# Alpha-VLLM/Lumina-T2X

Measured on AMD Instinct MI355X. Metric: denoising-steps/s & latent-tokens/s, Next-DiT 2B 1024^2 CFG, higher is better.
Workload: dtype bf16

## Files before the change

### include/lumina_dit_debug.h

```cpp
#ifndef LUMINA_DIT_DEBUG_H
#define LUMINA_DIT_DEBUG_H

#include "lumina_dit.h"

#ifdef __cplusplus
extern "C" {
#endif


int lt_op_attention_trace(const void* q_dev, const void* k_dev, const void* vt_dev, void* out_dev, int32_t B,
                          int32_t H, int32_t Hkv, int32_t N, int32_t Nk, int32_t Nkpad, int32_t hd, float scale,
                          void* trace_dev, void* stream);

int lt_op_rmsnorm_mod_ex(const void* x, const void* w, const void* scale, const void* shift, int32_t ld_mod, void* out, int32_t B,
                         int32_t N, int32_t d, float eps, int32_t scale_pre, int32_t out_pair, void* stream);
int lt_op_gated_residual_norm_ex(void* x, const void* y, const void* post_w, const void* gate, int32_t post_mode, int32_t gate_mode,
                                 const void* next_w, const void* next_scale, const void* next_shift, int32_t next_mode, int32_t ld_mod,
                                 void* h, int32_t B, int32_t N, int32_t d, float eps, float eps_next, int32_t scale_pre, int32_t h_pair,
                                 const void* ystat, int32_t ystat_slots, const void* moe_ys, const void* moe_pos, const void* moe_wts,
                                 const void* route_w, int32_t route_E, void* route_sel, void* route_wts, const void* route_forced,
                                 void* stream);
int lt_op_gated_residual_norm_describe(int32_t post_mode, int32_t gate_mode, int32_t next_mode, int32_t d, int32_t has_next_w,
                                       int32_t has_next_scale, int32_t has_next_shift, int32_t scale_pre, int32_t has_ystat,
                                       int32_t ystat_slots, int32_t has_moe, char* out, int32_t cap);
// ... 9 lines not shown
int lt_op_qkv_post(const void* qkv, int32_t ld, int32_t q_col0, int32_t k_col0, int32_t v_col0, const void* q_ln_w, const void* q_ln_b,
                   const void* k_ln_w, const void* k_ln_b, float ln_eps, void* q_dst, void* k_dst, void* vt_dst, int32_t B, int32_t N,
                   int32_t Npad, int32_t heads, int32_t kv_heads, int32_t hd, int32_t rope_mode, const void* cs_table, int32_t cs_len,
                   const void* t, float watershed, int32_t grid_w, const void* n_tok_b, const void* grid_w_b, float q_out_scale,
                   float k_out_scale, void* stream);

int lt_op_rk_stage(const void* y_dev, const void* const* k_ptrs_host, const float* coef_host, int32_t nk, float dt, void* out_dev, int64_t n,
                   int32_t dtype, void* stream);
int lt_op_rk_error_norm(const void* y_dev, const void* y1_dev, const void* const* k_ptrs_host, const float* coef_host, int32_t nk, float dt,
                        float rtol, float atol, void* q_dev, void* ws_dev, float* norm_dev, int64_t n, int32_t dtype, void* stream);
int lt_op_rk_dense(const void* y_dev, const void* y1_dev, const void* ymid_dev, const void* fy_dev, const void* f1_dev, float dt, void* c1_dev,
                   void* c_dev, void* b_dev, void* a_dev, int64_t n, int32_t dtype, void* stream);
int lt_op_rk_interp(const void* const* coef_ptrs_host, float x, void* out_dev, int64_t n, int32_t dtype, void* stream);
int lt_op_rms_norm(const void* x_dev, const void* sub_dev, const void* y0_dev, float rtol, float atol, void* q_dev, void* ws_dev, float* norm_dev,
                   int64_t n, int32_t dtype, void* stream);

int lt_op_patchify(const void* x, int32_t x_dtype, void* out, int32_t B, int32_t C, int32_t H, int32_t W, int32_t patch, int32_t kpad,
                   int32_t dup_first_half, int32_t wp_stride, void* stream);
int lt_op_eol_fill(void* x, const void* eol, int32_t rows_total, int32_t Wp, int32_t d, void* stream);
int lt_op_fill_rows_bf16(void* dst, const void* row, int64_t rows, int32_t d, void* stream);
int lt_op_label_gather(const void* table, const void* labels, void* out, int32_t B, int32_t rows, int32_t d, void* stream);
int lt_op_cast_to_bf16(const void* src, int32_t dtype, void* dst, int64_t n, void* stream);
int lt_op_upload_rows(const void* src, int32_t dtype, void* dst, int32_t rows, int32_t cols, int32_t dst_ld, int32_t r0, int32_t row_map,
                      void* stream);
int lt_op_mask_to_bias(const void* mask, void* bias, int32_t B, int32_t T, int32_t Tpad, void* stream);
int lt_op_add_bf16(const void* a, const void* b, void* c, int64_t n, void* stream);
int lt_op_timestep_features(const void* t, int32_t t_index, void* out, int32_t B, int32_t dim, void* stream);
int lt_op_cap_pool_ln(const void* cap, int32_t cap_dtype, const void* mask, const void* ln_w, const void* ln_b, void* out, int32_t B, int32_t T,
                      int32_t C, void* stream);
int lt_op_unpatchify_cfg(const void* rows, int32_t ld, void* out, int32_t out_dtype, int32_t B, int32_t C, int32_t out_ch, int32_t H, int32_t W,
                         int32_t patch, int32_t use_cfg, float cfg_scale, int32_t cfg_channels, int32_t wp_stride, void* stream);
int lt_op_unpatchify_cfg_dev(const void* rows, int32_t ld, void* out, int32_t out_dtype, int32_t B, int32_t C, int32_t out_ch, int32_t H, int32_t W,
                             int32_t patch, int32_t use_cfg, const float* cfg_scale_dev, int32_t cfg_channels, int32_t wp_stride, int32_t dup,
                             void* stream);
int32_t lt_op_guidance_slices(void);
int lt_op_guidance_stats(const void* rows, int32_t ld, int32_t B, int32_t out_ch, int32_t H, int32_t W, int32_t patch, const float* cfg_scale_dev,
                         int32_t cfg_channels, int32_t wp_stride, double* partials_dev, void* stream);
int lt_op_unpatchify_cfg_rule(const void* rows, int32_t ld, void* out, int32_t out_dtype, int32_t B, int32_t C, int32_t out_ch, int32_t H, int32_t W,
                              int32_t patch, int32_t use_cfg, const float* cfg_scale_dev, int32_t cfg_channels, int32_t wp_stride, int32_t dup,
                              const double* partials_dev, const float* rescale_dev, const float* norm_limit_dev, float* factor_out_dev,
                              void* stream);
int lt_op_guidance_project_stats(const void* rows, int32_t ld, int32_t B, int32_t out_ch, int32_t H, int32_t W, int32_t patch, int32_t cfg_channels,
                                 int32_t wp_stride, int32_t form, const float* par_dev, float* mom_dev, double* partials_dev, void* stream);
int lt_op_unpatchify_cfg_project(const void* rows, int32_t ld, void* out, int32_t out_dtype, int32_t B, int32_t C, int32_t out_ch, int32_t H,
                                 int32_t W, int32_t patch, int32_t use_cfg, const float* cfg_scale_dev, int32_t cfg_channels, int32_t wp_stride,
                                 int32_t dup, int32_t form, const double* partials_dev, const float* par_dev, const float* mom_dev,
                                 float* coef_out_dev, void* stream);
int lt_op_unpatchify_cfg_reuse(const void* rows, int32_t ld, void* out, int32_t out_dtype, int32_t B, int32_t C, int32_t out_ch, int32_t H, int32_t W,
                               int32_t patch, const float* cfg_scale_dev, int32_t cfg_channels, int32_t wp_stride, void* delta_dev, int32_t mode,
                               void* stream);
int lt_op_unpatchify_cfg_slg(const void* rows, int32_t ld, void* out, int32_t out_dtype, int32_t B, int32_t C, int32_t out_ch, int32_t H, int32_t W,
                             int32_t patch, const float* cfg_scale_dev, const float* slg_scale_dev, int32_t cfg_channels, int32_t wp_stride,
                             void* skip_dev, int32_t mode, void* stream);
int lt_op_attention_identity(const void* src, int32_t ld_src, int32_t col0, void* out, int32_t B, int32_t N, int32_t H, int32_t Hkv, int32_t hd,
                             int32_t out_pair, void* stream);
int lt_debug_cache_read(lt_engine* e, int32_t which, void* dst_dev, int64_t n, void* stream);
int32_t lt_op_cache_ws_bytes(void);
int lt_op_cache_indicator(const void* h_dev, void* h_prev_dev, int64_t n, void* ws_dev, double* sums_dev, void* stream);
int lt_op_cache_residual_store(const void* xl_dev, const void* x0_dev, void* r_dev, int64_t n, void* stream);
int lt_op_cache_residual_apply(void* x_dev, const void* r_dev, const void* scale1p_dev, const void* shift_dev, int32_t ld_mod, void* h_dev, int32_t B,
                               int32_t N, int32_t d, void* stream);
int lt_op_packed_table(const int32_t* hw_host, int32_t B, int32_t C, int32_t patch, int32_t* table_host, int64_t* elems, int32_t* n_max);
int lt_op_patchify_packed(const void* x_flat, int32_t x_dtype, void* out, const int32_t* hw_host, void* tab_dev, int32_t B, int32_t C,
                          int32_t patch, int32_t kpad, int32_t N, int32_t dup_first_half, void* stream);
int lt_op_fill_pad_packed(void* x, const void* pad_token, const int32_t* hw_host, void* tab_dev, int32_t B, int32_t patch, int32_t N, int32_t d,
                          void* stream);
int lt_op_unpatchify_packed(const void* rows, int32_t ld, void* out_flat, int32_t out_dtype, const int32_t* hw_host, void* tab_dev, int32_t B,
                            int32_t C, int32_t out_ch, int32_t patch, int32_t N, int32_t use_cfg, float cfg_scale, int32_t cfg_channels,
                            void* stream);
int lt_op_region_text_combine(void* out, const void* txt, const void* gate, int32_t Y, int32_t N, int32_t H, int32_t hd, int32_t Hp, int32_t Wp,
                              int32_t h_split, int32_t w_split, void* stream);
int lt_op_ode_combine(int32_t mode, const void* y0, const void* k1, const void* k2, const void* k3, const void* k4, void* out, int32_t dtype,
                      float dt, int64_t n, void* stream);
int lt_op_ode_combine_masked(int32_t mode, const void* y0, const void* k1, const void* k2, const void* k3, const void* k4, const void* mask,
                             const void* x1, const void* noise, void* out, int32_t dtype, float dt, float t, float one_minus_t, int64_t n,
                             void* stream);
int lt_op_ode_multistep(const void* y_prev, const void* const* k, int32_t nslopes, const float* a, const float* b, int32_t has_corr, void* y_out,
                        void* p_out, int64_t n, int32_t dtype, void* stream);
int lt_op_rope_table(void* out, int32_t len, int32_t hd, int32_t step, float theta0, float lin0, float theta1, float lin1, int32_t lin_on_pos,
                     void* stream, void* out_t);
int lt_op_linear_small_m_ext(const void* a, const void* w, const void* b, void* y, int32_t M, int32_t N, int32_t K, int32_t act_in, const void* t,
                             const void* a2, int32_t pm_L, int32_t pm_chunks, int32_t pm_d, int32_t pm_final, uint32_t pm_tanh, uint32_t pm_scale,
                             void* stream);
int lt_op_moe_route(const void* x, const void* gate_w, const void* forced, int32_t rows, int32_t rows_per_sample, int32_t d, int32_t E, void* sel,
                    void* wts, int32_t max_tiles, void* stream);
int lt_op_moe_plan_ex(void* sel, const void* sample_logits, int32_t sample_ld, const void* forced, void* wts, int32_t rows,
                      int32_t rows_per_sample, int32_t E, void* pos, void* src, void* tile_expert, int32_t max_tiles, int32_t layers,
                      int64_t layer_stride_rows, int64_t layer_stride_src, int64_t layer_stride_tiles, void* stream);

int lt_op_attention_qraw_ex(const void* qkv_dev, int32_t ld, int32_t q_col0, const void* q_mean_rstd_dev, const void* q_ln_w_dev,
                            const void* q_ln_b_dev, const void* cs_table_dev, const void* cs_table_t_dev, int32_t table_len, int32_t grid_w,
                            const void* t_dev, float watershed, const void* k_dev, const void* vt_dev, const void* tk_dev, const void* tvt_dev,
                            const float* tbias_dev, const void* tgate_dev, int32_t Tk, int32_t Tkpad, void* out_dev, int32_t B, int32_t H,
                            int32_t Hkv, int32_t N, int32_t Nkpad, int32_t hd, void* stream);
int lt_op_attention_qraw_nk(const void* qkv_dev, int32_t ld, int32_t q_col0, const void* q_mean_rstd_dev, const void* q_ln_w_dev,
                            const void* q_ln_b_dev, const void* cs_table_dev, const void* cs_table_t_dev, int32_t table_len, int32_t grid_w,
                            const void* t_dev, float watershed, const void* k_dev, const void* vt_dev, const void* tk_dev, const void* tvt_dev,
                            const float* tbias_dev, const void* tgate_dev, int32_t Tk, int32_t Tkpad, void* out_dev, int32_t B, int32_t H,
                            int32_t Hkv, int32_t N, int32_t Nkpad, int32_t hd, const int32_t* nk_dev, void* stream);
int lt_op_attention_small(const void* qkv_dev, int32_t ld, int32_t q_col0, int32_t k_col0, int32_t v_col0, const void* rowstat_dev, int32_t slots,
                          int32_t q_slot0, int32_t q_nslot, int32_t k_slot0, int32_t k_nslot, const void* q_ln_w_dev, const void* q_ln_b_dev,
                          const void* k_ln_w_dev, const void* k_ln_b_dev, const void* cs_table_dev, int32_t table_len, int32_t grid_w,
                          const void* t_dev, float watershed, float k_scale, void* out_dev, int32_t B, int32_t H, int32_t Hkv, int32_t tokens,
                          int32_t hd, void* stream);

int lt_op_views_guided_gather(const void* y_dev, const void* guidance_dev, const void* noise_dev, const int32_t* perm_dev, const float* vsign_dev,
                              const float* isign_dev, const void* f0_dev, void* out_dev, float half_dt, const float* coef_host, int32_t V,
                              int32_t C, int32_t HW, int32_t dtype, void* stream);

#ifdef __cplusplus
}
#endif
#endif
```

### lumina-t2x_amd/_lib.py

```python
from __future__ import annotations

import ctypes as C
import os
import re
from typing import Dict, List

_HERE = os.path.dirname(os.path.abspath(__file__))
LIB_PATH = os.environ.get("LUMINA_DIT_LIB") or os.path.join(_HERE, "lib", "liblumina_dit.so")
HEADER_PATH = os.path.join(os.path.dirname(_HERE), "include", "lumina_dit.h")
DEBUG_HEADER_PATH = os.path.join(os.path.dirname(_HERE), "include", "lumina_dit_debug.h")
LT_OPTION_INHERIT = -2 ** 31

LT_F32, LT_BF16, LT_F16 = 0, 1, 2
LT_VARIANT_NEXT_T2I, LT_VARIANT_NEXT_IMAGENET, LT_VARIANT_FLAG_T2I, LT_VARIANT_NEXT_MOE = 0, 1, 2, 3
LT_VARIANT_NEXT_MOE_TIME, LT_VARIANT_NEXT_MOE_SPACE = 4, 5
LT_SOFTMAX_T2I, LT_SOFTMAX_ANAGRAM = 0, 1
SOFTMAX_RULES = {"t2i": LT_SOFTMAX_T2I, "anagram": LT_SOFTMAX_ANAGRAM}
LT_PROJECT_APG, LT_PROJECT_ZERO_STAR = 1, 2
PROJECT_FORMS = {"apg": LT_PROJECT_APG, "zero_star": LT_PROJECT_ZERO_STAR}
LT_ODE_EULER, LT_ODE_MIDPOINT, LT_ODE_RK4 = 0, 1, 2
ODE_METHODS = {"euler": LT_ODE_EULER, "midpoint": LT_ODE_MIDPOINT, "rk4": LT_ODE_RK4}
LT_ODE_DOPRI5, LT_ODE_BOSH3, LT_ODE_FEHLBERG2, LT_ODE_ADAPTIVE_HEUN = 3, 4, 5, 6
ODE_ADAPTIVE_METHODS = {"dopri5": LT_ODE_DOPRI5, "bosh3": LT_ODE_BOSH3, "fehlberg2": LT_ODE_FEHLBERG2, "adaptive_heun": LT_ODE_ADAPTIVE_HEUN}
LT_ODE_AB2, LT_ODE_AB3, LT_ODE_ABM2, LT_ODE_ABM3 = 32, 33, 34, 35
# ... 125 lines not shown
    "lt_last_eval_rows": (_i64, [_vp]),
    "lt_graph_replays": (_i64, [_vp]),
    "lt_moe_routing_record": (_i32, [_vp, _i32]),
    "lt_moe_routing_read": (_i32, [_vp, C.POINTER(_i32), _i32]),
    "lt_moe_routing_force": (_i32, [_vp, C.POINTER(_i32), _i32]),
    "lt_profile_enable": (_i32, [_vp, _i32]),
    "lt_profile_read": (_i32, [_vp, _i32, C.POINTER(C.c_double), C.POINTER(_i64), C.POINTER(C.c_double)]),
    "lt_profile_reset": (_i32, [_vp]),
    "lt_profile_enable_mask": (_i32, [_vp, _i32]),
    "lt_profile_set_budget": (_i32, [_vp, _i32, _i64]),
    "lt_profile_set_window": (_i32, [_vp, _i32, _i64, _i64]),
    "lt_op_gemm_bf16": (_i32, [_vp, _vp, _vp, _i32, _vp, _i32, _i32, _i32, _i32, _i32, _vp]),
    "lt_op_pair_layout": (_i32, [_vp, _i64, _i32, _i32, _vp]),
    "lt_op_gemm_bf16_pair": (_i32, [_vp, _vp, _vp, _i32, _i32, _i32, _i32, _i32, _vp]),
    "lt_op_gemm_vt": (_i32, [_vp, _vp, _vp, _i32, _i32, _i32, _i32, _i32, _i32, _vp]),
    "lt_op_gemm_qkv": (_i32, [_vp, _vp, _vp, _vp, _i32, _i32, _i32, _i32, _i32, _i32, _vp]),
    "lt_op_gemm_qkv_fusable": (_i32, [_i32, _i32, _i32, _i32, _i32, _i32]),
    "lt_op_gemm_describe": (_i32, [_i32, _i32, _i32, _i32, _i32, C.c_char_p, _i32]),
    "lt_op_moe_plan": (_i32, [_vp, _vp, _vp, _i32, _i32, _i32, _vp, _vp, _vp, _i32, _vp]),
    "lt_op_gemm_splitk": (_i32, [_vp, _vp, _vp, _i32, _i32, _i32, _vp, _vp, _i32, _vp]),
    "lt_op_gemm_splitk_auto": (_i32, [_vp, _vp, _vp, _i32, _i32, _i32, _vp, _vp, _i32, _vp]),
    "lt_op_gemm_grouped": (_i32, [_vp, _vp, _vp, _i64, _vp, _i32, _i32, _i32, _i32, _i32, _vp]),
    "lt_op_gemm_grouped_tail": (_i32, [_vp, _vp, _vp, _i64, _vp, _i32, _i32, _i32, _vp, _vp, _i32, _vp]),
    "lt_op_gemm_grouped_gather": (_i32, [_vp, _i32, _vp, _vp, _vp, _i64, _vp, _i32, _i32, _i32, _i32, _i32, _vp]),
    "lt_op_pack_w13": (_i32, [_vp, _vp, _vp, _i32, _i32, _vp]),
    "lt_op_rmsnorm_mod": (_i32, [_vp, _vp, _vp, _vp, _i32, _vp, _i32, _i32, _i32, _f32, _i32, _vp]),
    "lt_op_gated_residual_norm": (_i32, [_vp, _vp, _vp, _vp, _i32, _i32, _vp, _vp, _vp, _i32, _i32, _vp, _i32, _i32, _i32, _f32, _f32, _i32, _vp]),
    "lt_op_prep_mod": (_i32, [_vp, _i32, _i32, _i32, _i32, _i32, C.c_uint32, C.c_uint32, _i32, _vp]),
    "lt_op_qk_norm_rope": (_i32, [_vp, _i32, _i32, _vp, _vp, _f32, _vp, _i32, _i32, _i32, _i32, _i32, _vp, _i32, _f32, _vp]),
    "lt_op_v_transpose": (_i32, [_vp, _i32, _i32, _vp, _i32, _i32, _i32, _i32, _i32, _vp]),
    "lt_op_attention_identity": (_i32, [_vp, _i32, _i32, _vp, _i32, _i32, _i32, _i32, _i32, _i32, _vp]),
    "lt_op_attention": (_i32, [_vp, _vp, _vp, _vp, _vp, _vp, _i32, _i32, _i32, _i32, _i32, _i32, _i32, _i32, _f32, _i32, _vp]),
    "lt_op_qkv_attention_small": (_i32, [_vp, _vp, _vp, _i32, _i32, _i32, _i32, _i32, _i32, _vp, _vp, _vp, _vp, _vp, _i32, _i32, _f32, _vp, _vp, _vp]),
    "lt_op_attention_describe": (_i32, [_i32, _i32, _i32, _i32, _i32, _i32, _i32, _i32, _i32, C.c_char_p, _i32]),
    "lt_op_attention_fused": (_i32, [_vp, _vp, _vp, _vp, _vp, _vp, _vp, _vp, _i32, _i32, _i32, _i32, _i32, _i32, _i32, _i32, _i32, _vp]),
    "lt_op_attention_nk": (_i32, [_vp, _vp, _vp, _vp, _vp, _vp, _i32, _i32, _i32, _i32, _i32, _i32, _i32, _i32, _f32, _i32, _vp, _i32, _vp]),
    "lt_op_attention_fused_nk": (_i32, [_vp, _vp, _vp, _vp, _vp, _vp, _vp, _vp, _i32, _i32, _i32, _i32, _i32, _i32, _i32, _i32, _i32, _vp, _i32, _vp]),
    "lt_op_attention_nk_describe": (_i32, [_i32, _i32, _i32, _i32, _i32, _i32, _i32, _i32, _i32, _i32, _i32, _i32, C.c_char_p, _i32]),
    "lt_op_attention_trace": (_i32, [_vp, _vp, _vp, _vp, _i32, _i32, _i32, _i32, _i32, _i32, _i32, _f32, _vp, _vp]),
    "lt_op_views_invert": (_i32, [_vp, _vp, _vp, _i32, _i32, _vp]),
    "lt_op_views_gather": (_i32, [_vp, _vp, _vp, _vp, _vp, _f32, _i32, _i32, _i32, _i32, _vp]),
    "lt_op_views_reduce": (_i32, [_vp, _vp, _vp, _vp, _vp, _f32, _i32, _i32, _i32, _i32, _vp]),
    "lt_op_windows_gather": (_i32, [_vp, C.POINTER(_i32), _i32, _i32, _i32, _i32, _i32, _vp, _i32, _i32, _vp]),
    "lt_op_windows_reduce": (_i32, [_vp, C.POINTER(_i32), _i32, _i32, _i32, _i32, _i32, _vp, _vp, _vp, _i32, _i32, _vp]),
    "lt_op_windows_cover": (_i32, [C.POINTER(_i32), _i32, _i32, _i32, _i32, _i32, _vp, _vp, _vp, _vp]),
    "lt_op_views_guided_gather": (_i32, [_vp, _vp, _vp, _vp, _vp, _vp, _vp, _vp, _f32, C.POINTER(_f32), _i32, _i32, _i32, _i32, _vp]),
    "lt_op_sde_step": (_i32, [_i32, _vp, _vp, _vp, _vp, _vp, _vp, _vp, C.POINTER(_f32), _i64, _i32, _vp]),
    "lt_op_rk_stage": (_i32, [_vp, C.POINTER(_vp), C.POINTER(_f32), _i32, _f32, _vp, _i64, _i32, _vp]),
    "lt_op_rk_error_norm": (_i32, [_vp, _vp, C.POINTER(_vp), C.POINTER(_f32), _i32, _f32, _f32, _f32, _vp, _vp, _vp, _i64, _i32, _vp]),
    "lt_op_rk_dense": (_i32, [_vp, _vp, _vp, _vp, _vp, _f32, _vp, _vp, _vp, _vp, _i64, _i32, _vp]),
    "lt_op_rk_interp": (_i32, [C.POINTER(_vp), _f32, _vp, _i64, _i32, _vp]),
    "lt_op_rms_norm": (_i32, [_vp, _vp, _vp, _f32, _f32, _vp, _vp, _vp, _i64, _i32, _vp]),
    "lt_op_linear_small_m": (_i32, [_vp, _vp, _vp, _vp, _i32, _i32, _i32, _i32, _vp]),
    "lt_op_patchify": (_i32, [_vp, _i32, _vp, _i32, _i32, _i32, _i32, _i32, _i32, _i32, _i32, _vp]),
    "lt_op_eol_fill": (_i32, [_vp, _vp, _i32, _i32, _i32, _vp]),
    "lt_op_fill_rows_bf16": (_i32, [_vp, _vp, _i64, _i32, _vp]),
    "lt_op_label_gather": (_i32, [_vp, _vp, _vp, _i32, _i32, _i32, _vp]),
    "lt_op_cast_to_bf16": (_i32, [_vp, _i32, _vp, _i64, _vp]),
    "lt_op_upload_rows": (_i32, [_vp, _i32, _vp, _i32, _i32, _i32, _i32, _i32, _vp]),
    "lt_op_mask_to_bias": (_i32, [_vp, _vp, _i32, _i32, _i32, _vp]),
    "lt_op_add_bf16": (_i32, [_vp, _vp, _vp, _i64, _vp]),
    "lt_op_timestep_features": (_i32, [_vp, _i32, _vp, _i32, _i32, _vp]),
    "lt_op_cap_pool_ln": (_i32, [_vp, _i32, _vp, _vp, _vp, _vp, _i32, _i32, _i32, _vp]),
    "lt_op_unpatchify_cfg_dev": (_i32, [_vp, _i32, _vp, _i32, _i32, _i32, _i32, _i32, _i32, _i32, _i32, _vp, _i32, _i32, _i32, _vp]),
    "lt_op_guidance_slices": (_i32, []),
    "lt_op_guidance_stats": (_i32, [_vp, _i32, _i32, _i32, _i32, _i32, _i32, _vp, _i32, _i32, _vp, _vp]),
    "lt_op_unpatchify_cfg_rule": (_i32, [_vp, _i32, _vp, _i32, _i32, _i32, _i32, _i32, _i32, _i32, _i32, _vp, _i32, _i32, _i32, _vp, _vp, _vp, _vp, _vp]),
    "lt_op_guidance_project_stats": (_i32, [_vp, _i32, _i32, _i32, _i32, _i32, _i32, _i32, _i32, _i32, _vp, _vp, _vp, _vp]),
    "lt_op_unpatchify_cfg_project": (_i32, [_vp, _i32, _vp, _i32, _i32, _i32, _i32, _i32, _i32, _i32, _i32, _vp, _i32, _i32, _i32, _i32, _vp, _vp, _vp,
                                            _vp, _vp]),
    "lt_op_unpatchify_cfg_reuse": (_i32, [_vp, _i32, _vp, _i32, _i32, _i32, _i32, _i32, _i32, _i32, _vp, _i32, _i32, _vp, _i32, _vp]),
    "lt_op_unpatchify_cfg_slg": (_i32, [_vp, _i32, _vp, _i32, _i32, _i32, _i32, _i32, _i32, _i32, _vp, _vp, _i32, _i32, _vp, _i32, _vp]),
    "lt_op_unpatchify_cfg": (_i32, [_vp, _i32, _vp, _i32, _i32, _i32, _i32, _i32, _i32, _i32, _i32, _f32, _i32, _i32, _vp]),
    "lt_op_packed_table": (_i32, [C.POINTER(_i32), _i32, _i32, _i32, C.POINTER(_i32), C.POINTER(_i64), C.POINTER(_i32)]),
    "lt_op_patchify_packed": (_i32, [_vp, _i32, _vp, C.POINTER(_i32), _vp, _i32, _i32, _i32, _i32, _i32, _i32, _vp]),
    "lt_op_fill_pad_packed": (_i32, [_vp, _vp, C.POINTER(_i32), _vp, _i32, _i32, _i32, _i32, _vp]),
    "lt_op_unpatchify_packed": (_i32, [_vp, _i32, _vp, _i32, C.POINTER(_i32), _vp, _i32, _i32, _i32, _i32, _i32, _i32, _f32, _i32, _vp]),
    "lt_op_region_text_combine": (_i32, [_vp, _vp, _vp, _i32, _i32, _i32, _i32, _i32, _i32, _i32, _i32, _vp]),
    "lt_op_ode_combine": (_i32, [_i32, _vp, _vp, _vp, _vp, _vp, _vp, _i32, _f32, _i64, _vp]),
    "lt_op_ode_combine_masked": (_i32, [_i32, _vp, _vp, _vp, _vp, _vp, _vp, _vp, _vp, _vp, _i32, _f32, _f32, _f32, _i64, _vp]),
    "lt_op_ode_multistep": (_i32, [_vp, C.POINTER(_vp), _i32, C.POINTER(_f32), C.POINTER(_f32), _i32, _vp, _vp, _i64, _i32, _vp]),
    "lt_op_rope_table": (_i32, [_vp, _i32, _i32, _i32, _f32, _f32, _f32, _f32, _i32, _vp, _vp]),
    "lt_op_linear_small_m_ext": (_i32, [_vp, _vp, _vp, _vp, _i32, _i32, _i32, _i32, _vp, _vp, _i32, _i32, _i32, _i32, C.c_uint32, C.c_uint32, _vp]),
    "lt_op_moe_route": (_i32, [_vp, _vp, _vp, _i32, _i32, _i32, _i32, _vp, _vp, _i32, _vp]),
    "lt_op_moe_plan_ex": (_i32, [_vp, _vp, _i32, _vp, _vp, _i32, _i32, _i32, _vp, _vp, _vp, _i32, _i32, _i64, _i64, _i64, _vp]),
    "lt_op_rope_table_2d": (_i32, [_vp, _i32, _i32, _f32, _f32, _vp]),
    "lt_op_rope_table_2d_pair": (_i32, [_vp, _vp, _i32, _i32, _f32, _f32, _vp]),
    "lt_op_proj_gated_residual_norm": (_i32, [_vp, _vp, _vp, _vp, _i32, _i32, _vp, _vp, _vp, _vp, _vp, _i32, _vp, _i32, _i32, _i32, _f32, _i32, _vp]),
    "lt_op_qkv_qstat": (_i32, [_vp, _vp, _vp, _vp, _i32, _i32, _i32, _i32, _i32, _i32, _i32, _vp, _vp, _vp, _i32, _f32, _vp, _vp, _vp, _vp]),
    "lt_op_attention_qraw": (_i32, [_vp, _i32, _i32, _vp, _vp, _vp, _vp, _vp, _i32, _i32, _vp, _vp, _vp, _i32, _i32, _i32, _i32, _i32, _i32, _vp]),
    "lt_op_attention_qraw_ex": (_i32, [_vp, _i32, _i32, _vp, _vp, _vp, _vp, _vp, _i32, _i32, _vp, _f32, _vp, _vp, _vp, _vp, _vp, _vp, _i32, _i32, _vp,
                                       _i32, _i32, _i32, _i32, _i32, _i32, _vp]),
    "lt_op_attention_qraw_nk": (_i32, [_vp, _i32, _i32, _vp, _vp, _vp, _vp, _vp, _i32, _i32, _vp, _f32, _vp, _vp, _vp, _vp, _vp, _vp, _i32, _i32, _vp,
                                       _i32, _i32, _i32, _i32, _i32, _i32, _vp, _vp]),
    "lt_op_attention_small": (_i32, [_vp, _i32, _i32, _i32, _i32, _vp, _i32, _i32, _i32, _i32, _i32, _vp, _vp, _vp, _vp, _vp, _i32, _i32, _vp, _f32,
                                     _f32, _vp, _i32, _i32, _i32, _i32, _i32, _vp]),
    "lt_op_rmsnorm_mod_ex": (_i32, [_vp, _vp, _vp, _vp, _i32, _vp, _i32, _i32, _i32, _f32, _i32, _i32, _vp]),
    "lt_op_gated_residual_norm_ex": (_i32, [_vp, _vp, _vp, _vp, _i32, _i32, _vp, _vp, _vp, _i32, _i32, _vp, _i32, _i32, _i32, _f32, _f32, _i32, _i32,
                                            _vp, _i32, _vp, _vp, _vp, _vp, _i32, _vp, _vp, _vp, _vp]),
    "lt_op_gated_residual_norm_describe": (_i32, [_i32, _i32, _i32, _i32, _i32, _i32, _i32, _i32, _i32, _i32, _i32, C.c_char_p, _i32]),
    "lt_op_qk_norm_rope_ex": (_i32, [_vp, _i32, _i32, _vp, _vp, _f32, _vp, _i32, _i32, _i32, _i32, _i32, _vp, _i32, _vp, _f32, _i32, _vp, _vp, _f32,
                                     _vp, _vp, _i32, _i32, _vp]),
    "lt_op_qk_norm_rope_pair": (_i32, [_vp, _i32, _i32, _i32, _vp, _vp, _vp, _vp, _f32, _vp, _vp, _i32, _i32, _i32, _i32, _i32, _i32, _vp, _i32, _vp,
                                       _f32, _i32, _vp, _vp, _f32, _f32, _vp]),
    "lt_op_qkv_post": (_i32, [_vp, _i32, _i32, _i32, _i32, _vp, _vp, _vp, _vp, _f32, _vp, _vp, _vp, _i32, _i32, _i32, _i32, _i32, _i32, _i32, _vp,
                              _i32, _vp, _f32, _i32, _vp, _vp, _f32, _f32, _vp]),
}

_lib = None


def load() -> C.CDLL:
    global _lib
    if _lib is not None:
        return _lib
    if not os.path.exists(LIB_PATH):
        raise LuminaLibError(
            f"HIP extension not built: {LIB_PATH} is missing. Run `python -c 'import __graft_entry__ as g; g.build()'` "
            "(or `make -C lumina-t2x_amd/csrc`). There is no CPU/PyTorch fallback for the denoising path."
        )
    try:
        lib = C.CDLL(LIB_PATH)
    except OSError as exc:
        raise LuminaLibError(f"cannot load {LIB_PATH}: {exc}") from exc
    for name, (res, args) in _SIGNATURES.items():
        try:
            fn = getattr(lib, name)
        except AttributeError as exc:
            raise LuminaLibError(f"{LIB_PATH} does not export {name}") from exc
        fn.restype = res
        fn.argtypes = args
    _lib = lib
    return lib


def check(rc: int, what: str = "") -> None:
    if rc != 0:
        msg = load().lt_last_error()
        raise LuminaLibError(f"{what or 'lumina_dit call'} failed (rc={rc}): {msg.decode() if msg else '?'}")
```

### lumina-t2x_amd/csrc/engine.h

```cpp
#pragma once
#include <map>
#include <string>
#include <vector>

#include "../../include/lumina_dit.h"
#include "common.h"
#include "eval_kind.h"
#include "kernels.h"
#include "options.h"

struct DevBuf {
    void* p = nullptr;
    size_t bytes = 0;
};

struct LayerW {
    u16 *wqkv = nullptr, *wo = nullptr, *w13 = nullptr, *w2 = nullptr, *wkvy = nullptr;
    u16 *q_norm_w = nullptr, *q_norm_b = nullptr, *k_norm_w = nullptr, *k_norm_b = nullptr;
    u16 *ky_norm_w = nullptr, *ky_norm_b = nullptr, *gate = nullptr;
    u16 *attn_norm1 = nullptr, *attn_norm2 = nullptr, *ffn_norm1 = nullptr, *ffn_norm2 = nullptr, *y_norm = nullptr;
    u16 *ky = nullptr, *vty = nullptr;
    u16 *w13_t = nullptr, *w2_t = nullptr, *w13_s = nullptr, *w2_s = nullptr, *gate_t = nullptr, *gate_s = nullptr;
    u16 *norm_time = nullptr, *norm_space = nullptr;
};

struct ProfClass {
    double flops = 0;
    long long launches = 0;
    std::vector<std::pair<hipEvent_t, hipEvent_t>> ev;
    size_t used = 0;
    size_t budget = (size_t)-1;
    long long skip = 0;
};

struct VariantDesc {
    int chunks;
    int i_shift[2], i_scale[2], i_gate[2];
    bool pre_w, post, gate_tanh, text, labels, rope_1d, eol;
    int final_chunks;
};

struct StageTimes {
    float *dev = nullptr, *pinned = nullptr;
    hipEvent_t copied = nullptr;
    int cap = 0;
    int reserve(int count) {
        LT_CHECK_HIP(hipMalloc((void**)&dev, (size_t)count * sizeof(float)));
        LT_CHECK_HIP(hipHostMalloc((void**)&pinned, (size_t)count * sizeof(float), hipHostMallocDefault));
        cap = count;
        return 0;
    }
    int create(int count) {
        if (reserve(count)) return 1;
        LT_CHECK_HIP(hipEventCreateWithFlags(&copied, hipEventDisableTiming));
        return 0;
    }
    void release() {
        if (dev) (void)hipFree(dev);
        if (pinned) (void)hipHostFree(pinned);
        if (copied) (void)hipEventDestroy(copied);
        dev = nullptr; pinned = nullptr; copied = nullptr; cap = 0;
    }
    int ready(int count, hipStream_t s) {
        if (cap < count) {
            LT_CHECK_HIP(hipStreamSynchronize(s));
            if (dev) LT_CHECK_HIP(hipFree(dev));
            if (pinned) LT_CHECK_HIP(hipHostFree(pinned));
            dev = nullptr; pinned = nullptr; cap = 0;
            if (reserve(count)) return 1;
        }
        LT_CHECK_HIP(hipEventSynchronize(copied));
        return 0;
    }
    float* begin(int count, hipStream_t s) { return ready(count, s) ? nullptr : pinned; }
    int commit(int count, hipStream_t s) {
        LT_CHECK_HIP(hipMemcpyAsync(dev, pinned, (size_t)count * sizeof(float), hipMemcpyHostToDevice, s));
        LT_CHECK_HIP(hipEventRecord(copied, s));
        return 0;
    }
};

struct RkWork {
    void *k[3] = {nullptr, nullptr, nullptr}, *coef[4] = {nullptr, nullptr, nullptr, nullptr}, *ws = nullptr;
    float *norm_dev = nullptr, *norm_host = nullptr;
    int reserve(size_t state_bytes) {
        if (norm_host) return 0;
        for (auto& p : k) LT_CHECK_HIP(hipMalloc(&p, state_bytes));
        for (auto& p : coef) LT_CHECK_HIP(hipMalloc(&p, state_bytes));
        LT_CHECK_HIP(hipMalloc(&ws, LT_RK_WS_BYTES));
        LT_CHECK_HIP(hipMalloc((void**)&norm_dev, 4 * sizeof(float)));
        LT_CHECK_HIP(hipHostMalloc((void**)&norm_host, 4 * sizeof(float), hipHostMallocDefault));
        return 0;
    }
    void release() {
        for (auto& p : k) { if (p) (void)hipFree(p); p = nullptr; }
        for (auto& p : coef) { if (p) (void)hipFree(p); p = nullptr; }
        if (ws) (void)hipFree(ws);
        if (norm_dev) (void)hipFree(norm_dev);
        if (norm_host) (void)hipHostFree(norm_host);
        ws = nullptr; norm_dev = nullptr; norm_host = nullptr;
    }
};

struct lt_engine {
    lt_config cfg;
    LtEngineOptions opts;
    VariantDesc v;
    int d, L, H, Hkv, hd, F, dkv, qkvn, A, cap, nfinal, kpad, chunks, ld_mod;
    std::vector<DevBuf> allocs;
    std::vector<LayerW> lw;
    u16 *xemb_w = nullptr, *xemb_b = nullptr, *t0_w = nullptr, *t0_b = nullptr, *t2_w = nullptr, *t2_b = nullptr;
    u16 *capln_w = nullptr, *capln_b = nullptr, *cape_w = nullptr, *cape_b = nullptr, *pad_token = nullptr;
    u16 *adaln_w = nullptr, *adaln_b = nullptr;
    u16 *final_w = nullptr, *final_b = nullptr;
    u16 *label_table = nullptr, *eol_token = nullptr;
    int label_rows = 0;
    std::map<std::string, bool> need;
    bool weights_ok = false;
    bool w_pair = false, last_pair = false;
    long long layout_flips_total = 0, layout_flips = 0;
    bool layout_pinned = false, w_owed = false;
    int* w_pair_dev = nullptr;
    u16 *x = nullptr, *h = nullptr, *qkv = nullptr, *q = nullptr, *k = nullptr, *vt = nullptr, *attn = nullptr;
    u16 *o = nullptr, *u = nullptr, *patches = nullptr, *frows = nullptr, *mod = nullptr;
    u16 *tfeat = nullptr, *t1 = nullptr, *temb = nullptr, *cap_ln = nullptr, *cap_emb = nullptr, *adaln_in = nullptr;
    int E = 0, moe_tiles = 0;
    int moe_mode = 0;
    u16 *moe_us = nullptr, *moe_ys = nullptr, *moe_logits = nullptr, *moe_wts = nullptr;
    u16* gate_t_all = nullptr;
    int *moe_sel = nullptr, *moe_pos = nullptr, *moe_tile_expert = nullptr, *moe_src = nullptr;
    int *moe_tp_sel = nullptr, *moe_tp_pos = nullptr, *moe_tp_tile_expert = nullptr, *moe_tp_src = nullptr;
    u16* moe_tp_wts = nullptr;
    size_t moe_tp_stride_rows = 0, moe_tp_stride_src = 0;
    bool moe_tp_live = false;
    int *moe_rec = nullptr, *moe_force = nullptr;
    int moe_rec_on = 0, moe_force_rows = 0, moe_rec_rows = 0;
    int qstat_slots = 32;
    float* qstat = nullptr;
    float* ystat = nullptr;
    int ystat_cap = 0;
    float* attn_tail_ws = nullptr;
    size_t attn_tail_ws_bytes = 0;
    float* qmr = nullptr;
    float* rope_tr = nullptr;
    float* splitk_part = nullptr;
    unsigned* splitk_cnt = nullptr;
    float* tail_part = nullptr;
    unsigned* tail_cnt = nullptr;
    long long tail_cap_parts = 0;
    int splitk_tiles = 0;
    u16 *capb = nullptr, *capn = nullptr, *kvy = nullptr;
    float* txt_bias = nullptr;
    float* rope = nullptr;
    float rope_scale = -1.f, rope_ntk = -1.f;
    int rope_len = 0;
    int prompt_B = 0, prompt_T = 0, prompt_Tpad = 0;
    int softmax_rule = LT_SOFTMAX_T2I;
    void *ys[2] = {nullptr, nullptr}, *ymid = nullptr, *kbuf[4] = {nullptr, nullptr, nullptr, nullptr};
    StageTimes times;
    RkWork rk;
    int reg_Y = 0, reg_h = 1, reg_w = 1;
    u16* reg_txt = nullptr;
    size_t reg_txt_elems = 0;
    int* reg_qmap = nullptr;
    int* pk_dev = nullptr;
    int pk_host[128] = {0};
    int* pk_tab = nullptr;
    long long last_nfe = 0;
    long long last_eval_rows = 0;
    int *vw_perm = nullptr, *vw_iperm = nullptr, *vw_hits = nullptr;
    float *vw_vsign = nullptr, *vw_isign = nullptr;
    int vw_V = 0, vw_h = 0, vw_w = 0;
    WindowTable tw = {};
    bool tw_has_weight = false;
    float *tw_weight = nullptr, *tw_wsum = nullptr;
    int* tw_bad = nullptr;
    void *tw_in = nullptr, *tw_out = nullptr;
    struct GraphTally { double flops[3] = {0, 0, 0}; long long launches[3] = {0, 0, 0}; };
    struct GraphEntry { std::vector<char> key; hipGraphExec_t exec = nullptr; int uses = 0; bool failed = false; bool pair = false; GraphTally tally; };
    GraphTally* tally = nullptr;
    std::vector<GraphEntry> graphs;
    void *g_x = nullptr, *g_out = nullptr;
    float* g_t = nullptr;
    float* g_cfg = nullptr;
    double* g_stats = nullptr;
    u16* g_delta = nullptr;
    int delta_sig[4] = {0, 0, 0, 0};
    u16* g_skip = nullptr;
    int rule_form = 0;
    float *p_mom = nullptr, *p_par = nullptr;
    double* p_stats = nullptr;
    int proj_sig[4] = {0, 0, 0, 0};
    std::vector<int32_t> skip;
    std::vector<int32_t> perturb;
    u16 *c_hprev = nullptr, *c_x0 = nullptr, *c_r = nullptr;
    double *c_ws = nullptr, *c_sums_host = nullptr;
    int cache_head[5] = {0, 0, 0, 0, 0}, cache_res[4] = {0, 0, 0, 0};
    long long last_cache_hits = 0;
    hipStream_t cap_stream = nullptr;
    long long graph_replays = 0;
    int prof_mask = 0;
    bool prof_on = false;
    ProfClass prof[3];
};

struct PackedCall {
    const int32_t* hw;
    long long elems;
    int n_max;
};
int packed_call_begin(lt_engine* e, const char* who, const int32_t* hw_host, const lt_step_args* a, int use_cfg, PackedCall* pc, hipStream_t s);
struct EvalSpec {
    LtEvalKind kind = LT_KIND_WHOLE;
    const PackedCall* pc = nullptr;
    const float* cfg_dev = nullptr;
};
int forward_graphed(lt_engine* e, const void* x_in, const float* t_dev, void* out, const lt_step_args* a, int use_cfg, hipStream_t s,
                    const EvalSpec& spec = {});
int ensure_step_cache(lt_engine* e);
int ensure_delta(lt_engine* e);
int ensure_skip_buf(lt_engine* e);
int ensure_project(lt_engine* e);
struct ProjectScope {
    lt_engine* e;
    ProjectScope(lt_engine* eng, int form) : e(eng) { e->rule_form = form; }
    ProjectScope(const ProjectScope&) = delete;
    ProjectScope& operator=(const ProjectScope&) = delete;
    ~ProjectScope() { e->rule_form = 0; }
};
struct SkipScope {
    lt_engine* e;
    explicit SkipScope(lt_engine* eng) : e(eng) {}
    SkipScope(const SkipScope&) = delete;
    SkipScope& operator=(const SkipScope&) = delete;
    ~SkipScope() { e->skip.clear(); e->perturb.clear(); }
    int set(const char* who, const int32_t* skip_host, int n_skip, const int32_t* perturb_host = nullptr, int n_perturb = 0);
};
int check_layer_sets(const lt_engine* e, const char* who, const int32_t* skip_host, int n_skip, const int32_t* perturb_host, int n_perturb);
int check_skip_set(const lt_engine* e, const char* who, const int32_t* skip_host, int n_skip);
bool stream_capturing(hipStream_t s);
int refuse_if_capturing(hipStream_t s, const char* who);
int refuse_profile_if_capturing(const lt_engine* e, hipStream_t s, const char* who);
int softmax_scale_for(const lt_engine* e, const lt_step_args* a, int N, float* scale);
void drop_views(lt_engine* e);
void drop_windows(lt_engine* e);
```

### lumina-t2x_amd/csrc/engine.hip

```cpp
#include <algorithm>
#include <cmath>
#include <cstdarg>
#include <cstdio>
#include <cstdlib>
#include <cstring>

#include "engine.h"
#include "kernels.h"

static thread_local char g_err[1024] = "";
void lt_set_error(const char* fmt, ...) {
    va_list ap;
    va_start(ap, fmt);
    vsnprintf(g_err, sizeof(g_err), fmt, ap);
    va_end(ap);
}
extern "C" const char* lt_last_error(void) { return g_err; }
extern "C" const char* lt_version(void) { return "lumina_dit gfx950 r5"; }

namespace {

constexpr float LOG2E = 1.44269504088896340736f;

VariantDesc variant_desc(int variant) {
// ... 373 lines not shown
    const lt_config& c = e->cfg; const VariantDesc& v = e->v;
    const LtEvalTraits kt = lt_eval_traits(kind);
    const int B = a->batch, p = c.patch_size;
    if (pk) {
        LT_REQUIRE(c.variant == LT_VARIANT_NEXT_T2I, "packed batches: the text-conditional Next-DiT (LT_VARIANT_NEXT_T2I) only; this engine is variant %d", c.variant);
        LT_REQUIRE(pk->tab || !use_cfg, "packed batches: lt_forward_packed is the plain forward (guidance on a size list: lt_forward_cfg_packed)");
        LT_REQUIRE(B >= 1 && B <= c.max_batch && B <= 64, "packed batch of %d exceeds max_batch %d (or 64)", B, c.max_batch);
    }
    LT_REQUIRE(B >= 1 && B <= c.max_batch, "batch %d exceeds max_batch %d", B, c.max_batch);
    LT_REQUIRE(!use_cfg || B % 2 == 0, "forward_with_cfg needs an even batch (cond+uncond)");
    LT_REQUIRE(a->latent_h % p == 0 && a->latent_w % p == 0, "latent %dx%d not divisible by patch", a->latent_h, a->latent_w);
    int Hp = a->latent_h / p, Wp = a->latent_w / p;
    dm.Wrow = v.eol ? Wp + 1 : Wp;
    int N = Hp * dm.Wrow;
    if (pk) {
        N = 0; Hp = 0; Wp = 0;
        for (int b = 0; b < B; ++b) {
            const int hb = pk->hw[2 * b], wb = pk->hw[2 * b + 1];
            LT_REQUIRE(hb > 0 && wb > 0 && hb % p == 0 && wb % p == 0, "packed sample %d: latent %dx%d not divisible by patch", b, hb, wb);
            dm.ntok[b] = (hb / p) * (wb / p);
            dm.gw[b] = wb / p;
            N = std::max(N, dm.ntok[b]); Hp = std::max(Hp, hb / p); Wp = std::max(Wp, wb / p);
        }
        for (int b = 0; b < B; ++b) dm.pk_full = dm.pk_full && dm.ntok[b] == N;
        dm.ntok_dev = pk->tab ? pk->tab + LT_PK_NTOK * LT_PK_MAX : e->pk_dev;
        dm.gw_dev = pk->tab ? pk->tab + LT_PK_GW * LT_PK_MAX : e->pk_dev + 64;
        dm.nk_dev = pk->tab && dm.pk_full ? nullptr : dm.ntok_dev;
    }
    dm.B = B; dm.N = N; dm.Npad = round_up(N, 64); dm.M = B * N; dm.Hp = Hp; dm.Wp = Wp;
    LT_REQUIRE(N <= c.max_tokens, "%d latent tokens exceed max_tokens %d", N, c.max_tokens);
    if (v.rope_1d) LT_REQUIRE(N <= e->rope_len, "sequence of %d tokens exceeds the 1-D RoPE table (%d)", N, e->rope_len);
    else LT_REQUIRE(Hp <= e->rope_len && Wp <= e->rope_len, "latent grid exceeds the RoPE table (%d)", e->rope_len);
    LT_REQUIRE(a->io_dtype == LT_BF16 || a->io_dtype == LT_F32, "io_dtype must be bf16 or f32");
    LT_REQUIRE(e->prompt_B == B || (kt.half && e->prompt_B == 2 * B), "%s was called for batch %d, step has batch %d",
               v.labels ? "lt_prepare_labels" : "lt_prepare_prompt", e->prompt_B, kt.half ? 2 * B : B);
    LT_REQUIRE(e->reg_Y == 0 || (B == 2 && !pk), "regional captions: one image per call (batch 2 = cond + uncond row), tensor input");
    LT_REQUIRE(e->skip.empty() || (!pk && (int)e->skip.size() < e->L), "layer skip: a tensor input and a set that leaves a layer (SkipScope::set)");
    LT_REQUIRE(e->skip.empty() || kt.skip_ok, "layer skip: a layer-skip set is not served by an evaluation of kind %d", (int)kind);
    LT_REQUIRE(e->perturb.empty() || !pk, "perturbed attention: a packed batch is not served (tensor input only)");
    LT_REQUIRE(e->perturb.empty() || kt.skip_ok, "perturbed attention: a perturb set is not served by an evaluation of kind %d", (int)kind);
    LT_REQUIRE(e->perturb.empty() || e->reg_Y == 0, "perturbed attention: a regional prompt is prepared (lt_prepare_prompt_regional), which is not served");
    if (lt_slg_kernel_mode(kind) >= 0) LT_REQUIRE(e->g_skip, "skip-layer guidance: the buffer is not allocated (ensure_skip_buf)");
    if (kind == LT_KIND_REUSE_STORE || kind == LT_KIND_REUSE_AGAIN) LT_REQUIRE(e->g_delta, "guidance reuse: the buffer is not allocated (ensure_delta)");
    LT_REQUIRE(e->rule_form == 0 || (kind == LT_KIND_RULE && e->p_mom && e->p_par && e->p_stats) || kind == LT_KIND_COND_ONLY,
               "projected guidance: form %d on an evaluation of kind %d, or the buffers are not allocated (ensure_project)", e->rule_form, (int)kind);
    e->cache_head[0] = 0;
    if (kt.cached) {
        LT_REQUIRE(!e->moe_rec_on && !e->moe_force_rows, "step caching: MoE routing record / force is not served");
        LT_REQUIRE(e->reg_Y == 0, "step caching: a regional prompt is not served");
        if (!e->tally && refuse_if_capturing(s, "step caching")) return 2;
        LT_REQUIRE(e->c_hprev && e->c_x0 && e->c_r && e->c_ws, "step caching: the buffers are not allocated (ensure_step_cache)");
    }
    if (!e->weights_ok && lt_weights_ready(e)) return 2;
    return 0;
}

int embed_patches(lt_engine* e, const Dims& dm, const void* x_in, const lt_step_args* a, int use_cfg, const PackedDesc* pk, hipStream_t s) {
    const lt_config& c = e->cfg;
    const int B = dm.B, N = dm.N, p = c.patch_size;
    if (ProfScope ps(e, 2, 0, s); !pk) {
        if (launch_patchify(x_in, a->io_dtype, e->patches, B, c.in_channels, a->latent_h, a->latent_w, p, e->kpad, use_cfg, dm.Wrow, s)) return 1;
    } else if (pk->tab) {
        if (launch_patchify_packed(pk->x_flat, a->io_dtype, e->patches, pk->tab, B, c.in_channels, p, e->kpad, N, use_cfg, s)) return 1;
    } else {
        for (int b = 0; b < B; ++b)
            if (launch_patchify(pk->x_ptrs[b], a->io_dtype, e->patches + (size_t)b * N * e->kpad, 1, c.in_channels, pk->hw[2 * b], pk->hw[2 * b + 1], p, e->kpad, 0, 0, s)) return 1;
        memcpy(e->pk_host, dm.ntok, B * sizeof(int)); memcpy(e->pk_host + 64, dm.gw, B * sizeof(int));
        LT_CHECK_HIP(hipMemcpyAsync(e->pk_dev, e->pk_host, 128 * sizeof(int), hipMemcpyHostToDevice, s));
    }
    if (gemm(e, e->patches, e->kpad, e->xemb_w, e->kpad, e->x, e->d, dm.M, e->d, e->kpad, e->xemb_b, 0, s)) return 1;
    if (pk) {
        ProfScope ps(e, 2, 0, s);
        if (pk->tab && !dm.pk_full && launch_fill_pad_packed(e->x, e->pad_token, pk->tab, B, N, e->d, s)) return 1;
        for (int b = 0; !pk->tab && b < B; ++b)
            if (dm.ntok[b] < N && launch_fill_rows_bf16(e->x + ((size_t)b * N + dm.ntok[b]) * e->d, e->pad_token, N - dm.ntok[b], e->d, s)) return 1;
    }
    if (e->v.eol) {
        ProfScope ps(e, 2, 0, s);
        if (launch_eol_fill(e->x, e->eol_token, B * dm.Hp, dm.Wp, e->d, s)) return 1;
    }
    return 0;
}

int condition(lt_engine* e, const Dims& dm, const float* t_dev, hipStream_t s) {
    const VariantDesc& v = e->v;
    const int B = dm.B, L = e->L, A = e->A;
    ProfScope ps(e, 2, 0, s);
    const int fused_pro = lt_opt(OPT_PROLOGUE_FUSED);
    if (fused_pro & 1) { LinearSmallMExtra x; x.t = t_dev; if (launch_linear_small_m_ext(nullptr, e->t0_w, e->t0_b, e->t1, B, A, 256, 0, x, s)) return 1; }
    else if (launch_timestep_features(t_dev, 0, e->tfeat, B, 256, s) || launch_linear_small_m(e->tfeat, e->t0_w, e->t0_b, e->t1, B, A, 256, 0, s)) return 1;
    if (launch_linear_small_m(e->t1, e->t2_w, e->t2_b, e->temb, B, A, A, 1, s)) return 1;
    if (e->gate_t_all && launch_linear_small_m(e->temb, e->gate_t_all, nullptr, e->moe_logits, B, L * e->E, A, 0, s)) return 1;
    if (e->moe_tp_live) {
        MoeArgs m;
        m.x = nullptr; m.gate_w = nullptr; m.forced = nullptr; m.sample_logits = e->moe_logits; m.sample_ld = L * e->E;
        m.rows = dm.M; m.rows_per_sample = dm.N; m.d = e->d; m.E = e->E;
        m.sel = e->moe_tp_sel; m.pos = e->moe_tp_pos; m.wts = e->moe_tp_wts; m.src = e->moe_tp_src; m.tile_expert = e->moe_tp_tile_expert;
        m.max_tiles = moe_tiles_for(e, dm.M);
        m.layers = L; m.layer_stride_rows = (long long)e->moe_tp_stride_rows; m.layer_stride_src = (long long)e->moe_tp_stride_src; m.layer_stride_tiles = e->moe_tiles;
        if (launch_moe_plan(m, s)) return 1;
    }
    unsigned tanh_mask = 0, scale_mask = 0;
    for (int i = 0; i < 2; ++i) {
        if (v.gate_tanh && v.i_gate[i] >= 0) tanh_mask |= 1u << v.i_gate[i];
        if (v.i_scale[i] >= 0) scale_mask |= 1u << v.i_scale[i];
    }
    if (e->cfg.variant == LT_VARIANT_NEXT_MOE) { tanh_mask |= 1u << 5; scale_mask |= 1u << 4; }
    const int fin2 = v.final_chunks == 2 ? 1 : 0;
    LinearSmallMExtra x;
    const u16* in = e->temb;
    if (fused_pro & 2) x.a2 = e->cap_emb;
    else { if (launch_add_bf16(e->temb, e->cap_emb, e->adaln_in, (long long)B * A, s)) return 1; in = e->adaln_in; }
    if (fused_pro & 4) { x.pm_L = L; x.pm_chunks = e->chunks; x.pm_d = e->d; x.pm_final = fin2; x.pm_tanh = tanh_mask; x.pm_scale = scale_mask; }
    if (fused_pro & 6 ? launch_linear_small_m_ext(in, e->adaln_w, e->adaln_b, e->mod, B, e->ld_mod, A, 1, x, s)
                      : launch_linear_small_m(in, e->adaln_w, e->adaln_b, e->mod, B, e->ld_mod, A, 1, s)) return 1;
    if (!(fused_pro & 4) && launch_prep_mod(e->mod, B, e->ld_mod, L, e->chunks, e->d, tanh_mask, scale_mask, fin2, s)) return 1;
    return 0;
}

bool fuses_text(const lt_engine* e) { return e->v.text && !(e->reg_Y > 0) && attention_fuses_text(e->hd); }
AttnArgs self_attn_args(const lt_engine* e, const Dims& dm, const LayerW& w) {
    AttnArgs at;
    at.q = e->q; at.k = e->k; at.vt = e->vt; at.bias = nullptr; at.out = e->attn; at.gate = nullptr; at.accumulate = 0;
    at.B = dm.B; at.H = e->H; at.Hkv = e->Hkv; at.N = dm.N; at.Nk = dm.N; at.Nkpad = dm.Npad; at.hd = e->hd; at.scale = dm.sm_scale; at.k_prescaled = 1;
    at.nk_batch = dm.nk_dev; at.tail_ws = e->attn_tail_ws; at.tail_ws_bytes = e->attn_tail_ws_bytes;
    if (fuses_text(e)) { at.tk = w.ky; at.tvt = w.vty; at.tbias = e->txt_bias; at.tgate = w.gate; at.Tk = e->prompt_T; at.Tkpad = e->prompt_Tpad; }
    return at;
}
GemmArgs qkv_gemm_args(const lt_engine* e, const Dims& dm, const LayerW& w) {
    GemmArgs gq;
    gq.A = e->h; gq.W = w.wqkv; gq.C = e->qkv; gq.bias = nullptr; gq.bias_dtype = -1; gq.M = dm.M; gq.N = e->d + 2 * e->dkv; gq.K = e->d;
    gq.lda = e->d; gq.ldw = e->d; gq.ldc = e->qkvn; gq.VT = e->vt; gq.vt_split = e->d + e->dkv; gq.vt_tokens = dm.N; gq.vt_hd = e->hd; gq.vt_npad = dm.Npad;
    return gq;
}

enum QkvRoute { QKV_SMALL_FUSED, QKV_FUSED, QKV_QK_AND_VT, QKV_PLAIN };
enum PostRoute { POST_K_ONLY, POST_ONE_LAUNCH, POST_QK_PAIR, POST_SEPARATE };
struct BlockPlan {
    bool regional, fuse_text;
    bool pk_one_wave;
    bool vt_epi;
    QkvRoute qkv;
    bool raw_q;
    int bn, qstat_slots;
    PostRoute post;
    bool pair;
    bool pair_moe;
};

int plan_block(const lt_engine* e, const Dims& dm, bool packed, BlockPlan& p) {
    const lt_config& c = e->cfg; const VariantDesc& v = e->v;
    const int M = dm.M, N = dm.N, d = e->d, dkv = e->dkv, hd = e->hd, F = e->F;
    const LayerW& w = e->lw[0];
    p = BlockPlan{}; p.regional = v.text && e->reg_Y > 0; p.fuse_text = fuses_text(e);
    const AttnArgs at = self_attn_args(e, dm, w);
    const GemmArgs gq = qkv_gemm_args(e, dm, w);
    p.pk_one_wave = packed && hd == 72 && N % 64 == 0 && attention_one_wave_hd72(at);
    p.vt_epi = lt_opt(OPT_QKV_VT_EPILOGUE) && (!packed || p.pk_one_wave) && N % 64 == 0 && (long long)((M + 255) / 256) * ((dkv + 255) / 256) >= 128;
    GemmArgs gs = gq;
    gs.VT = nullptr;
    const bool small_fused = lt_opt(OPT_ATTN_SMALL_FUSED) && !v.text && c.qk_norm && !v.rope_1d && !packed && !p.vt_epi &&
                             attention_small_fusable(hd, N, e->H, e->Hkv, d, dkv) && gemm_is_small_m(gs, 0);
    p.qkv = small_fused ? QKV_SMALL_FUSED : p.vt_epi && lt_opt(OPT_QKV_FUSED_GEMM) && gemm_qkv_fusable(gq) ? QKV_FUSED : p.vt_epi ? QKV_QK_AND_VT : QKV_PLAIN;
    if (p.qkv == QKV_FUSED) {
        p.bn = gemm_qkv_tile_width(gq);
        p.raw_q = lt_opt(OPT_ATTN_Q_FUSED) && c.qk_norm && !v.rope_1d && !packed && !p.regional && (p.fuse_text || !v.text) && attention_takes_raw_q(at) &&
                  p.bn > 0 && d % p.bn == 0 && 2 * d / p.bn <= 32;
        if (p.raw_q) p.qstat_slots = 2 * d / p.bn;
    }
    p.post = p.raw_q ? POST_K_ONLY
             : !p.vt_epi && (lt_opt(OPT_QKV_POST_FUSED) == 1 || (lt_opt(OPT_QKV_POST_FUSED) == 2 && M < 2048)) ? POST_ONE_LAUNCH
             : lt_opt(OPT_QK_POST_PAIR) && M >= 2048 ? POST_QK_PAIR : POST_SEPARATE;
    if (lt_opt(OPT_PAIR_LAYOUT) && e->E == 0 && (!packed || p.pk_one_wave) && M % 2 == 0 && d % 32 == 0 && F % 32 == 0 && F <= 16384 && d <= 16384 && !p.regional &&
        (!v.text || attention_fuses_text(hd))) {
        GemmArgs go, g13, g2;
        go.A = e->attn; go.W = w.wo; go.C = e->o; go.bias = nullptr; go.bias_dtype = -1; go.M = M; go.N = d; go.K = d; go.lda = d; go.ldw = d; go.ldc = d;
        g13 = go; g13.A = e->h; g13.W = w.w13; g13.C = e->u; g13.N = 2 * F; g13.ldc = F;
        g2 = go; g2.A = e->u; g2.W = w.w2; g2.K = F; g2.lda = F; g2.ldw = F;
        p.pair = p.qkv == QKV_FUSED && gemm_runs_w4q_dense(go, 0) && gemm_runs_w4q_dense(g13, 1) && gemm_runs_w4q_dense(g2, 0) && attention_is_one_wave(at);
    }
    if (lt_opt(OPT_PAIR_LAYOUT) && e->E > 0 && d % 32 == 0 && F % 32 == 0 && F <= 16384 && d <= 16384) {
        GemmArgs g13, g2;
        moe_gemm_args(e, w.w13_t ? w.w13_t : w.w13_s, w.w2_t ? w.w2_t : w.w2_s, e->moe_tile_expert, e->moe_src, M, g13, g2);
        p.pair_moe = gemm_runs_w4q_grouped(g13, 1) && gemm_runs_w4q_grouped(g2, 0);
    }
    if (e->layout_pinned) { p.pair = false; p.pair_moe = false; }
    LT_REQUIRE(!p.pair || (p.qkv == QKV_FUSED && !p.regional && (p.fuse_text || !v.text)), "pair layout: the block left the path it was chosen for");
    return 0;
}

struct PerturbPlan {
    bool text = false;
    int variant = 0, pair_ab = 0;
    bool out_pair = false;
    bool attn_rowmajor = false;
};
int plan_perturbed(const lt_engine* e, const BlockPlan& bp, PerturbPlan& pp) {
    pp = PerturbPlan{};
    pp.text = e->v.text;
    LT_REQUIRE(!bp.regional, "perturbed attention: a regional prompt is not served");
// ... 268 lines not shown
    if (!e->p_par) { if (dev_alloc(e, &q, 4 * sizeof(float))) return 1; e->p_par = (float*)q; }
    return 0;
}

int ensure_delta(lt_engine* e) { return ensure_half_state(e, &e->g_delta, "guidance reuse"); }
int ensure_skip_buf(lt_engine* e) { return ensure_half_state(e, &e->g_skip, "skip-layer guidance"); }

static int check_layer_set(const lt_engine* e, const char* who, const char* what, const int32_t* host, int n) {
    LT_REQUIRE(n >= 0, "%s: n_%s %d is negative", who, what, n);
    LT_REQUIRE(n == 0 || host, "%s: null argument (%s_host: %d layer indices)", who, what, n);
    LT_REQUIRE(n <= e->L, "%s: %d %s indices, the model has %d layers", who, n, what, e->L);
    for (int i = 0; i < n; ++i) {
        LT_REQUIRE(host[i] >= 0 && host[i] < e->L, "%s: %s index %d (entry %d) is outside 0..%d", who, what, host[i], i, e->L - 1);
        for (int j = 0; j < i; ++j) LT_REQUIRE(host[j] != host[i], "%s: %s index %d is repeated (entries %d and %d)", who, what, host[i], j, i);
    }
    return 0;
}

int check_layer_sets(const lt_engine* e, const char* who, const int32_t* skip_host, int n_skip, const int32_t* perturb_host, int n_perturb) {
    if (check_layer_set(e, who, "skip", skip_host, n_skip)) return 2;
    LT_REQUIRE(n_skip < e->L, "%s: the skip set leaves no layer (all %d are in it)", who, e->L);
    if (check_layer_set(e, who, "perturb", perturb_host, n_perturb)) return 2;
    for (int i = 0; i < n_perturb; ++i)
        for (int j = 0; j < n_skip; ++j)
            LT_REQUIRE(perturb_host[i] != skip_host[j], "%s: layer %d is in the skip set and in the perturb set (the sets are disjoint)", who, perturb_host[i]);
    return 0;
}

int check_skip_set(const lt_engine* e, const char* who, const int32_t* skip_host, int n_skip) {
    return check_layer_sets(e, who, skip_host, n_skip, nullptr, 0);
}

int SkipScope::set(const char* who, const int32_t* skip_host, int n_skip, const int32_t* perturb_host, int n_perturb) {
    if (check_layer_sets(e, who, skip_host, n_skip, perturb_host, n_perturb)) return 2;
    e->skip.assign(skip_host, skip_host + n_skip);
    std::sort(e->skip.begin(), e->skip.end());
    e->perturb.assign(perturb_host, perturb_host + n_perturb);
    std::sort(e->perturb.begin(), e->perturb.end());
    return 0;
}

int refuse_profile_if_capturing(const lt_engine* e, hipStream_t s, const char* who) {
    if (!(e->prof_on && e->prof_mask)) return 0;
    LT_REQUIRE(!stream_capturing(s), "%s: refused on a stream under capture while lt_profile_enable is on (the profile brackets launches with "
               "events, which a graph cannot carry): switch the profile off before the capture", who);
    return 0;
}

int softmax_scale_for(const lt_engine* e, const lt_step_args* a, int N, float* scale) {
    const int hd = e->hd;
    if (a->proportional_attn && !e->v.labels) {
        LT_REQUIRE(a->base_seqlen > 1, "proportional_attn needs base_seqlen");
        const double lg = std::log((double)N) / std::log((double)a->base_seqlen);
        if (e->softmax_rule == LT_SOFTMAX_ANAGRAM) {
            const long long chunks = (long long)((double)N / (double)a->base_seqlen + 0.99);
            LT_REQUIRE(chunks * a->base_seqlen >= N, "LT_SOFTMAX_ANAGRAM: %lld query chunks of base_seqlen %d do not cover %d tokens (the reference's "
                       "chunk loop drops the last %lld query rows at this shape)", chunks, a->base_seqlen, N, (long long)N - chunks * a->base_seqlen);
            *scale = (float)(lg / std::sqrt((double)hd));
        } else {
            *scale = (float)std::sqrt(lg / (double)hd);
        }
    } else {
        *scale = (float)std::sqrt(1.0 / (double)hd);
    }
    return 0;
}

static int forward_graphed_body(lt_engine* e, const void* x_in, const float* t_dev, void* out, const lt_step_args* a, int use_cfg, hipStream_t s,
                               const EvalSpec& spec) {
    const PackedCall* pc = spec.pc;
    const LtEvalKind kind = spec.kind;
    const LtEvalTraits kt = lt_eval_traits(kind);
    lt_step_args own;
    if (kt.dev_scale) {
        LT_REQUIRE(!pc && a->batch % 2 == 0, "a guidance schedule needs a tensor state with an even batch");
        own = *a;
        own.cfg_scale = 0.f;
        if (kt.half) own.batch = a->batch / 2;
        if (kind != LT_KIND_COND_ONLY && spec.cfg_dev != e->g_cfg)
            LT_CHECK_HIP(hipMemcpyAsync(e->g_cfg, spec.cfg_dev, sizeof(float), hipMemcpyDeviceToDevice, s));
        a = &own;
        use_cfg = kt.half ? 0 : 1;
    }
    auto run = [&](const void* x, const float* t, void* o, hipStream_t st) {
        if (!pc) return run_forward(e, x, t, o, a, use_cfg, st, nullptr, kind);
        PackedDesc pk{nullptr, nullptr, pc->hw};
        pk.x_flat = x; pk.out_flat = o; pk.tab = e->pk_tab;
        return run_forward(e, nullptr, t, nullptr, a, use_cfg, st, &pk);
    };
    if (!lt_opt(OPT_GRAPH) || profiling_wants_events(e) || e->moe_rec_on || e->moe_force_rows) return run(x_in, t_dev, out, s);
    const int B = a->batch;
    if (lt_opt(OPT_GRAPH) == 2 && pc && (long long)B * pc->n_max <= 1024) return run(x_in, t_dev, out, s);
    if (lt_opt(OPT_GRAPH) == 2 && !pc && a->latent_h > 0 && a->latent_w > 0 && e->cfg.patch_size > 0 &&
        (long long)B * (a->latent_h / e->cfg.patch_size) * (a->latent_w / e->cfg.patch_size) <= 1024)
        return run(x_in, t_dev, out, s);
    if (B < 1 || B > e->cfg.max_batch || (!pc && (a->latent_h <= 0 || a->latent_w <= 0)) || (a->io_dtype != LT_BF16 && a->io_dtype != LT_F32))
        return run(x_in, t_dev, out, s);
    const size_t sbytes = (pc ? (size_t)pc->elems : (size_t)B * e->cfg.in_channels * a->latent_h * a->latent_w) * (a->io_dtype == LT_BF16 ? 2 : 4);
    const size_t cap_bytes = (size_t)e->cfg.max_batch * e->cfg.in_channels * e->cfg.max_tokens * e->cfg.patch_size * e->cfg.patch_size * 4;
    if ((kt.half ? 2 * sbytes : sbytes) > cap_bytes) return run(x_in, t_dev, out, s);
    if (stream_capturing(s)) return run(x_in, t_dev, out, s);
    const int extra[11] = {use_cfg, e->prompt_B, e->prompt_T, e->prompt_Tpad, e->reg_Y, e->reg_h, e->reg_w, lt_opt_generation(), lt_opt_engine_generation(),
                           e->softmax_rule, (int)kind};
    std::vector<char> key(sizeof(lt_step_args) + sizeof(extra));
    memcpy(key.data(), a, sizeof(lt_step_args));
    memcpy(key.data() + sizeof(lt_step_args), extra, sizeof(extra));
    if (pc) key.insert(key.end(), (const char*)pc->hw, (const char*)(pc->hw + 2 * B));
    if (!e->skip.empty()) {
        const int32_t mark[2] = {-1, (int32_t)e->skip.size()};
        key.insert(key.end(), (const char*)mark, (const char*)(mark + 2));
        key.insert(key.end(), (const char*)e->skip.data(), (const char*)(e->skip.data() + e->skip.size()));
    }
    if (!e->perturb.empty()) {
        const int32_t mark[2] = {-2, (int32_t)e->perturb.size()};
        key.insert(key.end(), (const char*)mark, (const char*)(mark + 2));
        key.insert(key.end(), (const char*)e->perturb.data(), (const char*)(e->perturb.data() + e->perturb.size()));
    }
    if (e->rule_form != 0 && kind == LT_KIND_RULE) {
        const int32_t mark[2] = {-3, (int32_t)e->rule_form};
        key.insert(key.end(), (const char*)mark, (const char*)(mark + 2));
    }
    lt_engine::GraphEntry* ge = nullptr;
    for (auto& g : e->graphs) if (g.key == key) { ge = &g; break; }
    if (!ge) {
        if (e->graphs.size() >= 16) {
            if (e->graphs.front().exec) (void)hipGraphExecDestroy(e->graphs.front().exec);
            e->graphs.erase(e->graphs.begin());
        }
        e->graphs.emplace_back();
        ge = &e->graphs.back();
        ge->key = key;
    }
    if (e->layout_pinned && ge->pair) {
        if (ge->exec) (void)hipGraphExecDestroy(ge->exec);
        ge->exec = nullptr; ge->uses = 0; ge->failed = false; ge->pair = false;
    }
    if (ge->failed || ge->uses++ == 0) {
        const int rc = run(x_in, t_dev, out, s);
        ge->pair = e->last_pair;
        return rc;
    }
    if (ensure_rope(e, a, s)) return 1;
    if (ensure_weight_layout(e, ge->pair, s)) return 1;
    if (!ge->exec) {
        if (!e->cap_stream) LT_CHECK_HIP(hipStreamCreateWithFlags(&e->cap_stream, hipStreamNonBlocking));
        hipGraph_t graph = nullptr;
        bool ok = hipStreamBeginCapture(e->cap_stream, hipStreamCaptureModeThreadLocal) == hipSuccess;
        int rc = 0;
        if (ok) {
            ge->tally = lt_engine::GraphTally();
            e->tally = &ge->tally;
            rc = run(e->g_x, e->g_t, e->g_out, e->cap_stream);
            e->tally = nullptr;
            if (rc == 0 && e->last_pair != ge->pair) { lt_set_error("graph capture: the evaluation's operand layout changed between the eager run and the capture"); rc = 1; }
            ok = hipStreamEndCapture(e->cap_stream, &graph) == hipSuccess && rc == 0 && graph != nullptr;
        }
        if (ok) ok = hipGraphInstantiate(&ge->exec, graph, nullptr, nullptr, 0) == hipSuccess;
        if (graph) (void)hipGraphDestroy(graph);
        if (!ok) {
            (void)hipGetLastError();
            ge->exec = nullptr;
            ge->failed = true;
            if (rc) return rc;
            return run(x_in, t_dev, out, s);
        }
    }
    if (kt.reads_x) LT_CHECK_HIP(hipMemcpyAsync(e->g_x, x_in, sbytes, hipMemcpyDeviceToDevice, s));
    LT_CHECK_HIP(hipMemcpyAsync(e->g_t, t_dev, (size_t)B * sizeof(float), hipMemcpyDeviceToDevice, s));
    LT_CHECK_HIP(hipGraphLaunch(ge->exec, s));
    e->last_pair = ge->pair;
    if (kt.writes_out)
        LT_CHECK_HIP(hipMemcpyAsync(out, e->g_out, kt.half ? 2 * sbytes : sbytes, hipMemcpyDeviceToDevice, s));
    ++e->graph_replays;
    if (e->prof_on)
        for (int k = 0; k < 3; ++k)
            if ((e->prof_mask >> k) & 1) { e->prof[k].flops += ge->tally.flops[k]; e->prof[k].launches += ge->tally.launches[k]; }
    return 0;
}

int forward_graphed(lt_engine* e, const void* x_in, const float* t_dev, void* out, const lt_step_args* a, int use_cfg, hipStream_t s,
                    const EvalSpec& spec) {
    const int sig[5] = {a->batch, a->latent_h, a->latent_w, a->io_dtype, use_cfg};
    if (lt_eval_traits(spec.kind).cached) {
        LT_REQUIRE(!spec.pc, "step caching: a packed batch is not served (tensor input only)");
        LT_REQUIRE(spec.kind == LT_KIND_CACHE_HEAD || memcmp(e->cache_head, sig, sizeof sig) == 0, "step caching: this evaluation does not follow "
                   "its probe - the head of an evaluation of the same step arguments, with no other evaluation between");
    }
    e->cache_head[0] = 0;
    const int rc = forward_graphed_body(e, x_in, t_dev, out, a, use_cfg, s, spec);
    if (rc == 0 && spec.kind == LT_KIND_CACHE_HEAD) memcpy(e->cache_head, sig, sizeof sig);
    return rc;
}

int ensure_step_cache(lt_engine* e) {
    if (e->c_sums_host) return 0;
    const size_t words = (size_t)e->cfg.max_batch * e->cfg.max_tokens * e->d;
    void* q = nullptr;
    if (!e->c_hprev) { if (dev_alloc(e, &q, words * sizeof(u16))) return 1; e->c_hprev = (u16*)q; }
    if (!e->c_x0) { if (dev_alloc(e, &q, words * sizeof(u16), false)) return 1; e->c_x0 = (u16*)q; }
    if (!e->c_r) { if (dev_alloc(e, &q, words * sizeof(u16), false)) return 1; e->c_r = (u16*)q; }
    if (!e->c_ws) { if (dev_alloc(e, &q, (2 * LT_CACHE_BLOCKS + 2) * sizeof(double))) return 1; e->c_ws = (double*)q; }
    LT_CHECK_HIP(hipHostMalloc((void**)&e->c_sums_host, 2 * sizeof(double), hipHostMallocDefault));
    return 0;
}

extern "C" int lt_create(const lt_config* cfg, lt_engine** out) {
    LT_REQUIRE(cfg && out, "lt_create: null argument");
    LT_REQUIRE(cfg->variant >= LT_VARIANT_NEXT_T2I && cfg->variant <= LT_VARIANT_NEXT_MOE_SPACE, "lt_create: unknown variant %d", cfg->variant);
    const bool is_moe = cfg->variant == LT_VARIANT_NEXT_MOE || cfg->variant == LT_VARIANT_NEXT_MOE_TIME || cfg->variant == LT_VARIANT_NEXT_MOE_SPACE;
    LT_REQUIRE(!is_moe || (cfg->num_experts >= 2 && cfg->num_experts <= 8),
               "lt_create: the MoE variant needs 2..8 experts (top-2 routing), got %d", cfg->num_experts);
    const VariantDesc vd = variant_desc(cfg->variant);
    LT_REQUIRE(cfg->dim > 0 && cfg->n_layers >= 1 && cfg->n_heads >= 1 && cfg->n_kv_heads >= 1 && cfg->ffn_hidden > 0 && cfg->adaln_dim > 0,
               "lt_create: dim, n_layers, n_heads, n_kv_heads, ffn_hidden and adaln_dim must be positive");
    LT_REQUIRE(cfg->patch_size >= 1 && cfg->in_channels >= 1 && cfg->out_channels >= 1 && cfg->max_tokens >= 1 && cfg->max_text >= 0,
               "lt_create: patch_size, in_channels, out_channels, max_tokens must be positive (max_text >= 0)");
    LT_REQUIRE(cfg->dim % cfg->n_heads == 0, "dim %% n_heads != 0");
    LT_REQUIRE(cfg->n_heads % cfg->n_kv_heads == 0, "n_heads %% n_kv_heads != 0");
    const int hd = cfg->dim / cfg->n_heads;
    LT_REQUIRE(hd == 48 || hd == 72 || hd == 96 || hd == 128, "head_dim %d not built (48, 72, 96, 128)", hd);
    LT_REQUIRE(hd != 128 || !vd.text, "head_dim 128 with text cross-attention not built (the class-conditional and MoE variants run at head_dim 128)");
    LT_REQUIRE(cfg->dim % 64 == 0 && cfg->ffn_hidden % 64 == 0, "dim and ffn_hidden must be multiples of 64");
    LT_REQUIRE(!vd.text || (cfg->cap_feat_dim % 64 == 0 && cfg->cap_feat_dim > 0), "cap_feat_dim must be a positive multiple of 64");
    LT_REQUIRE(!vd.labels || cfg->num_classes > 0, "class-conditional variant needs num_classes > 0");
    LT_REQUIRE(cfg->dim <= 4096 && cfg->cap_feat_dim <= 4096, "dim / cap_feat_dim above 4096 not supported by the row kernels");
    LT_REQUIRE(cfg->adaln_dim % 8 == 0 && cfg->max_batch >= 1 && cfg->max_batch <= 8, "adaln_dim %% 8 and 1 <= max_batch <= 8 required");
    LT_REQUIRE(cfg->in_channels * cfg->patch_size * cfg->patch_size <= 64, "patch vector longer than 64");
    lt_engine* e = new lt_engine();
    e->cfg = *cfg;
    e->v = vd;
    e->d = cfg->dim; e->L = cfg->n_layers; e->H = cfg->n_heads; e->Hkv = cfg->n_kv_heads; e->hd = hd;
    e->F = cfg->ffn_hidden; e->dkv = e->Hkv * hd; e->qkvn = e->d + 2 * e->dkv; e->A = cfg->adaln_dim;
    e->cap = vd.text ? cfg->cap_feat_dim : 0; e->nfinal = cfg->patch_size * cfg->patch_size * cfg->out_channels;
    e->kpad = 64; e->chunks = vd.chunks; e->ld_mod = e->L * e->chunks * e->d + vd.final_chunks * e->d;
    e->label_rows = vd.labels ? cfg->num_classes + 1 : 0;
    e->E = is_moe ? cfg->num_experts : 0;
    e->moe_mode = cfg->variant == LT_VARIANT_NEXT_MOE_TIME ? 1 : (cfg->variant == LT_VARIANT_NEXT_MOE_SPACE ? 2 : 0);
    e->rope_len = vd.rope_1d ? round_up(cfg->max_tokens, 64) : (cfg->rope_table_len > 0 ? cfg->rope_table_len : 384);
    const int d = e->d, L = e->L, F = e->F, dkv = e->dkv, A = e->A, cap = e->cap, H = e->H, Hkv = e->Hkv;
    e->lw.resize(L);
    auto fail = [&]() { lt_destroy(e); return 1; };
#define A16(ptr, n) do { void* _p; if (dev_alloc(e, &_p, (size_t)(n) * 2)) return fail(); (ptr) = (u16*)_p; } while (0)
    const int Tmax = round_up(cfg->max_text > 0 ? cfg->max_text : 64, 64);
    for (int l = 0; l < L; ++l) {
        LayerW& w = e->lw[l];
        A16(w.wqkv, (size_t)e->qkvn * d); A16(w.wo, (size_t)d * d);
        if (e->E == 0) { A16(w.w13, (size_t)2 * F * d); A16(w.w2, (size_t)d * F); }
        else {
            const size_t E_ = e->E;
            if (e->moe_mode != 2) {
                A16(w.w13_t, E_ * 2 * F * d); A16(w.w2_t, E_ * d * F);
                if (l == 0) A16(e->gate_t_all, (size_t)L * E_ * A);
                w.gate_t = e->gate_t_all + (size_t)l * E_ * A;
            }
            if (e->moe_mode != 1) { A16(w.w13_s, E_ * 2 * F * d); A16(w.w2_s, E_ * d * F); A16(w.gate_s, E_ * d); }
            A16(w.norm_time, d); A16(w.norm_space, d);
        }
        A16(w.q_norm_w, d); A16(w.q_norm_b, d); A16(w.k_norm_w, dkv); A16(w.k_norm_b, dkv);
        A16(w.attn_norm1, d); A16(w.attn_norm2, d); A16(w.ffn_norm1, d); A16(w.ffn_norm2, d);
        if (vd.text) {
            A16(w.wkvy, (size_t)2 * dkv * cap); A16(w.ky_norm_w, dkv); A16(w.ky_norm_b, dkv); A16(w.gate, H); A16(w.y_norm, cap);
            A16(w.ky, (size_t)cfg->max_batch * Hkv * Tmax * hd); A16(w.vty, (size_t)cfg->max_batch * Hkv * hd * Tmax);
        }
        char key[128];
        std::vector<const char*> names = {"attention.wq.weight", "attention.wk.weight", "attention.wv.weight", "attention.wo.weight",
                                          "adaLN_modulation.1.weight", "adaLN_modulation.1.bias"};
        if (e->E == 0) for (const char* nm : {"feed_forward.w1.weight", "feed_forward.w2.weight", "feed_forward.w3.weight"}) names.push_back(nm);
        if (vd.text) for (const char* nm : {"attention.wk_y.weight", "attention.wv_y.weight", "attention.gate", "attention_y_norm.weight"}) names.push_back(nm);
        if (cfg->variant == LT_VARIANT_NEXT_T2I)
            for (const char* nm : {"attention_norm1.weight", "attention_norm2.weight", "ffn_norm1.weight", "ffn_norm2.weight"}) names.push_back(nm);
        else if (cfg->variant == LT_VARIANT_NEXT_MOE)
            for (const char* nm : {"attention_norm.weight", "ffn_norm_time.weight", "ffn_norm_space.weight",
                                   "feed_forward_time.gate.weight", "feed_forward_space.gate.weight"}) names.push_back(nm);
        else if (e->moe_mode != 0)
// ... 583 lines not shown
```

### lumina-t2x_amd/csrc/kernels.h

```cpp
#pragma once
#include <hip/hip_runtime.h>
#include <stdint.h>
#include "common.h"

struct GemmArgs {
    const u16* A;
    const u16* W;
    u16* C;
    const void* bias;
    int M, N, K;
    int lda, ldw, ldc;
    int bias_dtype;
    unsigned long long* trace = nullptr;
    const int* tile_expert = nullptr;
    long long w_expert_stride = 0;
    const int* a_row_map = nullptr;
    int a_map_rows = 0;
    int vt_tokens = 0, vt_hd = 0, vt_npad = 0;
    u16* VT = nullptr;
    int vt_split = 0;
    float* splitk_part = nullptr;
    unsigned* splitk_cnt = nullptr;
    int splitk_tiles = 0;
    int split_k = 0;
// ... 124 lines not shown
    size_t tail_ws_bytes = 0;
    int out_pair = 0;
    unsigned long long* trace = nullptr;
    const u16* q_raw = nullptr;
    int q_ld = 0, q_col0 = 0;
    const float* q_stat = nullptr;
    const u16* q_ln_w = nullptr;
    const u16* q_ln_b = nullptr;
    const float* rope_cs = nullptr;
    const float* rope_cs_t = nullptr;
    const float* rope_t = nullptr;
    float rope_watershed = 0.f;
    int rope_cs_len = 0, rope_grid_w = 0;
    const int* nk_batch = nullptr;
    const int* q_batch_map = nullptr;
};
int launch_region_text_combine(u16* out, const u16* txt, const u16* gate, int Y, int N, int H, int hd, int Hp, int Wp,
                               int h_split, int w_split, hipStream_t stream);
int launch_attention(const AttnArgs& a, hipStream_t stream);
bool attention_one_wave_hd72(const AttnArgs& a);
struct AttnSmallArgs {
    const u16* qkv;
    int ld, q_col0, k_col0, v_col0;
    const float* rowstat;
    int slots, q_slot0, q_nslot, k_slot0, k_nslot;
    const u16 *q_ln_w, *q_ln_b, *k_ln_w, *k_ln_b;
    float ln_eps;
    const float* cs;
    const float* t;
    float watershed;
    int cs_len, grid_w;
    float k_scale;
    u16* out;
    int B, H, Hkv, N, hd;
    PrefetchRider pf;
};
bool attention_small_fusable(int hd, int N, int H, int Hkv, int q_width, int k_width);
int launch_attention_small(const AttnSmallArgs& a, hipStream_t stream);
int launch_attention_v4(const AttnArgs& a, hipStream_t stream);
int launch_attention_v4_hd48(const AttnArgs& a, hipStream_t stream);
int launch_attention_v4_hd96(const AttnArgs& a, hipStream_t stream);
int launch_attention_hd128(const AttnArgs& a, hipStream_t stream);
bool attention_takes_hd128_fast(const AttnArgs& a);
const char* attention_describe(const AttnArgs& a);
size_t attention_tail_ws_floats(int heads, int parts, int rows);
bool attention_is_one_wave(const AttnArgs& a);
bool attention_takes_raw_q(const AttnArgs& a);
bool attention_fuses_text(int hd);
int ensure_dynamic_lds(const void* fn, int bytes);
bool gemm_runs_w4q_grouped(const GemmArgs& a, int epilogue);
bool gemm_runs_w4q_dense(const GemmArgs& a, int epilogue);
const char* lt_gemm_describe(const GemmArgs& a, int epilogue, int variant);

struct MoeArgs {
    const u16* x;
    const u16* gate_w;
    const u16* sample_logits;
    int sample_ld = 0;
    const int* forced;
    int rows, rows_per_sample, d, E;
    int* sel;
    u16* wts;
    int* pos;
    int* src;
    int* tile_expert;
    int max_tiles;
    int layers = 1;
    long long layer_stride_rows = 0, layer_stride_src = 0, layer_stride_tiles = 0;
};
constexpr int LT_MOE_PLAN_TIME_MAX_SAMPLES = 64;
int launch_moe_route(const MoeArgs& a, hipStream_t stream);
int launch_moe_plan(const MoeArgs& a, hipStream_t stream);

int launch_linear_small_m(const u16* a, const u16* w, const u16* b, u16* y, int M, int N, int K, int act_in,
                          hipStream_t stream);
struct LinearSmallMExtra {
    const float* t = nullptr;
    const u16* a2 = nullptr;
    int pm_L = 0, pm_chunks = 0, pm_d = 0, pm_final = -1;
    unsigned pm_tanh = 0, pm_scale = 0;
};
int launch_linear_small_m_ext(const u16* a, const u16* w, const u16* b, u16* y, int M, int N, int K, int act_in,
                              const LinearSmallMExtra& x, hipStream_t stream);
int launch_cast_to_bf16(const void* src, int dtype, u16* dst, long long n, hipStream_t stream);
int launch_patchify(const void* x, int x_dtype, u16* out, int B, int C, int H, int W, int patch, int kpad,
                    int dup_first_half, int wp_stride, hipStream_t stream);
int launch_eol_fill(u16* x, const u16* eol, int rows_total, int Wp, int d, hipStream_t stream);
int launch_label_gather(const u16* table, const int32_t* labels, u16* out, int B, int rows, int d, hipStream_t stream);
int launch_timestep_features(const float* t, int t_index, u16* out, int B, int dim, hipStream_t stream);
int launch_cap_pool_ln(const void* cap, int cap_dtype, const int32_t* mask, const u16* ln_w, const u16* ln_b,
                       u16* out, int B, int T, int C, hipStream_t stream);
int launch_prep_mod(u16* mod, int B, int ld_mod, int L, int chunks, int d, unsigned tanh_mask, unsigned scale_mask,
                    int final_scale_chunk, hipStream_t stream);
int launch_add_bf16(const u16* a, const u16* b, u16* c, long long n, hipStream_t stream);
int launch_mask_to_bias(const int32_t* mask, float* bias, int B, int T, int Tpad, hipStream_t stream);
int launch_unpatchify_cfg(const u16* rows, int ld, void* out, int out_dtype, int B, int C, int out_ch, int H, int W,
                          int patch, int use_cfg, float cfg_scale, int cfg_channels, int wp_stride, hipStream_t stream);
int launch_unpatchify_cfg_dev(const u16* rows, int ld, void* out, int out_dtype, int B, int C, int out_ch, int H, int W, int patch, int use_cfg,
                              const float* cfg_scale_dev, int cfg_channels, int wp_stride, int dup, hipStream_t stream);
constexpr int LT_GUIDANCE_SLICES = 32;
int launch_guidance_stats(const u16* rows, int ld, int B, int out_ch, int H, int W, int patch, const float* cfg_scale_dev, int cfg_channels,
                          int wp_stride, double* partials, hipStream_t stream);
int launch_unpatchify_cfg_rule(const u16* rows, int ld, void* out, int out_dtype, int B, int C, int out_ch, int H, int W, int patch, int use_cfg,
                               const float* cfg_scale_dev, int cfg_channels, int wp_stride, int dup, const double* partials,
                               const float* rescale_dev, const float* limit_dev, float* factor_out, hipStream_t stream);
int launch_guidance_params_store(float* dst, float scale, float rescale, float limit, hipStream_t stream);
constexpr int LT_PROJECT_SUMS = 3;
int launch_guidance_project_stats(const u16* rows, int ld, int B, int out_ch, int H, int W, int patch, int cfg_channels, int wp_stride, int form,
                                  const float* par_dev, float* mom, double* partials, hipStream_t stream);
int launch_unpatchify_cfg_project(const u16* rows, int ld, void* out, int out_dtype, int B, int C, int out_ch, int H, int W, int patch, int use_cfg,
                                  const float* cfg_scale_dev, int cfg_channels, int wp_stride, int dup, int form, const double* partials,
                                  const float* par_dev, const float* mom, float* coef_out, hipStream_t stream);
int launch_guidance_project_params_store(float* dst, float scale, float eta, float beta, float r, hipStream_t stream);
int launch_unpatchify_cfg_reuse(const u16* rows, int ld, void* out, int out_dtype, int B, int C, int out_ch, int H, int W, int patch,
                                const float* cfg_scale_dev, int cfg_channels, int wp_stride, u16* delta, int mode, hipStream_t stream);
int launch_unpatchify_cfg_slg(const u16* rows, int ld, void* out, int out_dtype, int B, int C, int out_ch, int H, int W, int patch,
                              const float* cfg_scale_dev, const float* slg_scale_dev, int cfg_channels, int wp_stride, u16* skip, int mode,
                              hipStream_t stream);
int launch_slg_params_store(float* g_cfg, float cfg_scale, float slg_scale, hipStream_t stream);
constexpr int LT_CACHE_BLOCKS = 512;
int launch_cache_indicator(const u16* h, u16* h_prev, long long n, double* partials, double* sums, hipStream_t stream);
int launch_cache_residual_store(const u16* xl, const u16* x0, u16* r, long long n, hipStream_t stream);
int launch_cache_residual_apply(u16* x, const u16* r, const u16* scale, const u16* shift, int ld_mod, u16* h, int rows, int rows_per_batch, int d,
                                hipStream_t stream);
int launch_ode_combine(int mode, const void* y0, const void* k1, const void* k2, const void* k3, const void* k4,
                       void* out, int dtype, float dt, long long n, hipStream_t stream);
int launch_ode_combine_masked(int mode, const void* y0, const void* k1, const void* k2, const void* k3, const void* k4, const void* mask,
                              const void* x1, const void* noise, void* out, int dtype, float dt, float t, float one_minus_t, long long n,
                              hipStream_t stream);
int multistep_used(const float* c);
int launch_ode_multistep(const void* y_prev, const void* const* k, int nslopes, const float* a, const float* b, int has_corr, void* y_out,
                         void* p_out, long long n, int dtype, hipStream_t stream);
int launch_views_invert(const int* perm, int* iperm, int* hits, int V, int HW, hipStream_t stream);
int launch_views_gather(const void* y, const int* perm, const float* vsign, const void* f0, void* out, float half_dt, int V, int C, int HW,
                        int dtype, hipStream_t stream);
int launch_views_reduce(const void* y, const void* f, const int* iperm, const float* isign, void* out, float dt, int V, int C, int HW, int dtype,
                        hipStream_t stream);
int launch_views_guided_gather(const void* y, const void* guidance, const void* noise, const int* perm, const float* vsign, const float* isign,
                               const void* f0, void* out, float half_dt, const float* coef, int V, int C, int HW, int dtype, hipStream_t stream);
#define LT_WINDOWS_MAX 64
struct WindowTable {
    int n, win_h, win_w, canvas_h, canvas_w;
    int off[2 * LT_WINDOWS_MAX];
};
int window_table_build(const char* who, const int32_t* offsets_host, int n, int win_h, int win_w, int canvas_h, int canvas_w, WindowTable* out);
int launch_windows_gather(const void* y, const WindowTable& t, void* out, int C, int dtype, hipStream_t stream);
int launch_windows_cover(const WindowTable& t, const float* weight, float* wsum, int* bad, hipStream_t stream);
int launch_windows_reduce(const void* f, const WindowTable& t, const float* weight, const float* wsum, void* out, int C, int dtype,
                          hipStream_t stream);
int launch_sde_step(int op, const void* x, const void* v, const void* w, const void* k1, const void* xp, void* out, void* out2, const float* rec,
                    long long n, int dtype, hipStream_t stream);
int launch_flowedit_mix(const void* x_src, const void* z, const void* noise, void* out4, float t, float omt, long long n_half, int dtype,
                        hipStream_t stream);
int launch_flowedit_combine(const void* z, const void* out4, void* z_next, float w_s, float w_t, float dt, int Bp, int C, int HW, int ch, int dtype,
                            hipStream_t stream);
int launch_rk_stage(const void* y, const void* const* k, const float* coef, int nk, float dt, void* out, long long n, int dtype,
                    hipStream_t stream);
int launch_rk_error_norm(const void* y, const void* y1, const void* const* k, const float* c_err, int nk, float dt, float rtol, float atol,
                         void* q_out, void* ws, float* norm_out, long long n, int dtype, hipStream_t stream);
int launch_rms_norm(const void* x, const void* sub, const void* y0, float rtol, float atol, void* q_out, void* ws, float* norm_out, long long n,
                    int dtype, hipStream_t stream);
int launch_rk_dense(const void* y, const void* y1, const void* ymid, const void* fy, const void* f1, float dt, void* c1, void* c, void* b, void* a,
                    long long n, int dtype, hipStream_t stream);
int launch_rk_interp(const void* const* coeffs, float x, void* out, long long n, int dtype, hipStream_t stream);
int launch_upload_rows(const void* src, int dtype, u16* dst, int rows, int cols, int dst_ld, int r0, int row_map,
                       hipStream_t stream);
// ... 16 lines not shown
```

### lumina-t2x_amd/csrc/misc.hip

```cpp
#include "common.h"
#include "kernels.h"

namespace {

constexpr int SM_MAXM = 8;
constexpr int SM_NC = 8;
template <int MM, bool EXT = false>
__global__ __launch_bounds__(256) void linear_small_m_kernel(const u16* __restrict__ a, const u16* __restrict__ w,
                                                             const u16* __restrict__ bias, u16* __restrict__ y, int M,
                                                             int N, int K, int act_in, LinearSmallMExtra x = LinearSmallMExtra()) {
    const int lane = threadIdx.x & 63;
    const int n0 = (blockIdx.x * 4 + (threadIdx.x >> 6)) * SM_NC;
    if (n0 >= N) return;
    const int nch = K >> 3;
    float acc[SM_NC][MM];
#pragma unroll
    for (int j = 0; j < SM_NC; ++j)
#pragma unroll
        for (int m = 0; m < MM; ++m) acc[j][m] = 0.f;
    for (int c = lane; c < nch; c += 64) {
        bf8_t wv[SM_NC];
#pragma unroll
        for (int j = 0; j < SM_NC; ++j) {
            const int n = n0 + j < N ? n0 + j : N - 1;
            wv[j] = *(const bf8_t*)(w + (size_t)n * K + c * 8);
        }
        float af[MM][8];
#pragma unroll
        for (int m = 0; m < MM; ++m) {
            if (m < M) {
                if (EXT && x.t) {
                    const int half = K / 2;
#pragma unroll
                    for (int e = 0; e < 8; ++e) {
                        const int k = c * 8 + e, kk = k < half ? k : k - half;
                        const float freq = expf(-9.210340371976184f * (float)kk / (float)half);
                        const float arg = x.t[m] * freq;
                        af[m][e] = bfr(k < half ? cosf(arg) : sinf(arg));
                    }
                } else {
                    unpack8(*(const bf8_t*)(a + (size_t)m * K + c * 8), af[m]);
                }
                if (EXT && x.a2) {
                    float bf_[8];
                    unpack8(*(const bf8_t*)(x.a2 + (size_t)m * K + c * 8), bf_);
#pragma unroll
                    for (int e = 0; e < 8; ++e) af[m][e] = bfr(af[m][e] + bf_[e]);
                }
                if (act_in == 1) {
#pragma unroll
                    for (int e = 0; e < 8; ++e) af[m][e] = bfr(silu_f(af[m][e]));
                }
            } else {
#pragma unroll
                for (int e = 0; e < 8; ++e) af[m][e] = 0.f;
            }
        }
#pragma unroll
        for (int j = 0; j < SM_NC; ++j) {
            float wf[8];
            unpack8(wv[j], wf);
#pragma unroll
            for (int m = 0; m < MM; ++m)
#pragma unroll
                for (int e = 0; e < 8; ++e) acc[j][m] += af[m][e] * wf[e];
        }
    }
#pragma unroll
    for (int j = 0; j < SM_NC; ++j) {
        if (n0 + j < N) {
#pragma unroll
            for (int m = 0; m < MM; ++m) {
                if (m < M) {
                    float s = wave_sum(acc[j][m]);
                    if (lane == 0) {
                        if (bias) s += bf2f(bias[n0 + j]);
                        u16 o = f2bf(s);
                        if (EXT && x.pm_d > 0) {
                            const int n = n0 + j, layers = x.pm_L * x.pm_chunks * x.pm_d;
                            int mode = 0;
                            if (n < layers) {
                                const int ch = (n / x.pm_d) % x.pm_chunks;
// ... 59 lines not shown
    if (i >= B * d) return;
    const int b = i / d, c = i % d;
    int l = labels[b];
    l = l < 0 ? 0 : (l >= rows ? rows - 1 : l);
    out[i] = table[(size_t)l * d + c];
}

__global__ void timestep_features_kernel(const float* __restrict__ t, u16* __restrict__ out, int B, int dim) {
    const int half = dim / 2;
    const int i = blockIdx.x * blockDim.x + threadIdx.x;
    if (i >= B * half) return;
    const int b = i / half, k = i % half;
    const float freq = expf(-9.210340371976184f * (float)k / (float)half);
    const float arg = t[b] * freq;
    out[(size_t)b * dim + k] = f2bf(cosf(arg));
    out[(size_t)b * dim + half + k] = f2bf(sinf(arg));
}

__global__ __launch_bounds__(256) void cap_pool_ln_kernel(const void* __restrict__ cap, int cap_dtype,
                                                          const int32_t* __restrict__ mask, const u16* __restrict__ ln_w,
                                                          const u16* __restrict__ ln_b, u16* __restrict__ out, int T, int C) {
    extern __shared__ float sh[];
    float* pooled = sh;
    float* red = sh + C;
    const int b = blockIdx.x;
    float cnt = 0.f;
    for (int t = 0; t < T; ++t) cnt += (float)mask[b * T + t];
    for (int c = threadIdx.x; c < C; c += blockDim.x) {
        float s = 0.f;
        for (int t = 0; t < T; ++t) {
            const size_t idx = ((size_t)b * T + t) * C + c;
            const float v = cap_dtype == 0 ? ((const float*)cap)[idx] : bf2f(((const u16*)cap)[idx]);
            s += v * (float)mask[b * T + t];
        }
        s = s / cnt;
        pooled[c] = cap_dtype == 0 ? s : bfr(s);
    }
    __syncthreads();
    float s = 0.f;
    for (int c = threadIdx.x; c < C; c += blockDim.x) s += pooled[c];
    s = wave_sum(s);
    if ((threadIdx.x & 63) == 0) red[threadIdx.x >> 6] = s;
    __syncthreads();
    const float mean = (red[0] + red[1] + red[2] + red[3]) / (float)C;
    __syncthreads();
    float q = 0.f;
    for (int c = threadIdx.x; c < C; c += blockDim.x) {
        const float d = pooled[c] - mean;
        q += d * d;
    }
    q = wave_sum(q);
    if ((threadIdx.x & 63) == 0) red[threadIdx.x >> 6] = q;
    __syncthreads();
    const float rstd = rsqrtf((red[0] + red[1] + red[2] + red[3]) / (float)C + 1e-5f);
    for (int c = threadIdx.x; c < C; c += blockDim.x)
        out[(size_t)b * C + c] = f2bf((pooled[c] - mean) * rstd * bf2f(ln_w[c]) + bf2f(ln_b[c]));
}

__global__ void prep_mod_kernel(u16* __restrict__ mod, int B, int ld_mod, int L, int chunks, int d, unsigned tanh_mask,
                                unsigned scale_mask, int final_scale_chunk) {
    const long long per_b = (long long)L * chunks * d + (final_scale_chunk >= 0 ? d : 0);
    const long long total = (long long)B * per_b;
    for (long long i = (long long)blockIdx.x * blockDim.x + threadIdx.x; i < total; i += (long long)gridDim.x * blockDim.x) {
        const int b = (int)(i / per_b);
        const long long r = i % per_b;
        u16* p;
        int mode;
        if (r < (long long)L * chunks * d) {
            const int ch = (int)((r / d) % chunks);
            mode = ((tanh_mask >> ch) & 1u) ? 1 : (((scale_mask >> ch) & 1u) ? 2 : 0);
            p = mod + (size_t)b * ld_mod + r;
        } else {
            mode = 2;
            p = mod + (size_t)b * ld_mod + (size_t)L * chunks * d + (size_t)final_scale_chunk * d + (r - (long long)L * chunks * d);
        }
        if (mode == 1) *p = f2bf(tanhf(bf2f(*p)));
        else if (mode == 2) *p = f2bf(1.0f + bf2f(*p));
    }
}

__global__ void add_bf16_kernel(const u16* a, const u16* b, u16* c, long long n) {
    const long long i = (long long)blockIdx.x * blockDim.x + threadIdx.x;
    if (i < n) c[i] = f2bf(bf2f(a[i]) + bf2f(b[i]));
}

__global__ void mask_to_bias_kernel(const int32_t* mask, float* bias, int B, int T, int Tpad) {
    const int i = blockIdx.x * blockDim.x + threadIdx.x;
    if (i >= B * Tpad) return;
    const int b = i / Tpad, t = i % Tpad;
    bias[i] = (t < T && mask[b * T + t] != 0) ? 0.f : -INFINITY;
}

__global__ void unpatchify_cfg_kernel(const u16* __restrict__ rows, int ld, void* __restrict__ out, int out_dtype, int B,
                                      int C, int out_ch, int H, int W, int patch, int use_cfg, float cfg_scale,
                                      int cfg_channels, int wp_stride) {
#pragma clang fp contract(off)
    const long long total = (long long)B * C * H * W;
    const int Hp = H / patch;
    for (long long i = (long long)blockIdx.x * blockDim.x + threadIdx.x; i < total; i += (long long)gridDim.x * blockDim.x) {
        const int w = (int)(i % W);
        const int hh = (int)((i / W) % H);
        const int c = (int)((i / ((long long)W * H)) % C);
        const int b = (int)(i / ((long long)W * H * C));
        const int e = ((hh % patch) * patch + (w % patch)) * out_ch + c;
        const long long tok = (long long)(hh / patch) * wp_stride + (w / patch);
        auto rd = [&](int bb) { return bf2f(rows[((long long)bb * Hp * wp_stride + tok) * ld + e]); };
        float v;
        if (use_cfg && c < cfg_channels) {
            const int half = B / 2;
            const int bc = b % half;
            const float cond = rd(bc), unc = rd(bc + half);
            v = bfr(unc + bfr(cfg_scale * bfr(cond - unc)));
        } else {
            v = rd(b);
        }
        if (out_dtype == 0) ((float*)out)[i] = v;
        else ((u16*)out)[i] = f2bf(v);
    }
}

__global__ void unpatchify_cfg_dev_kernel(const u16* __restrict__ rows, int ld, void* __restrict__ out, int out_dtype, int B, int C, int out_ch,
                                          int H, int W, int patch, int use_cfg, const float* __restrict__ cfg_scale_dev, int cfg_channels,
                                          int wp_stride, int dup) {
#pragma clang fp contract(off)
    const long long total = (long long)B * C * H * W;
    const int Hp = H / patch;
    const int half = B / 2;
    const float cfg_scale = (use_cfg && !dup) ? cfg_scale_dev[0] : 0.f;
    for (long long i = (long long)blockIdx.x * blockDim.x + threadIdx.x; i < total; i += (long long)gridDim.x * blockDim.x) {
        const int w = (int)(i % W);
        const int hh = (int)((i / W) % H);
        const int c = (int)((i / ((long long)W * H)) % C);
        const int b = (int)(i / ((long long)W * H * C));
        const int e = ((hh % patch) * patch + (w % patch)) * out_ch + c;
        const long long tok = (long long)(hh / patch) * wp_stride + (w / patch);
        auto rd = [&](int bb) { return bf2f(rows[((long long)bb * Hp * wp_stride + tok) * ld + e]); };
        float v;
        if (dup) {
            v = rd(b % half);
        } else if (use_cfg && c < cfg_channels) {
            const int bc = b % half;
            const float cond = rd(bc), unc = rd(bc + half);
            v = bfr(unc + bfr(cfg_scale * bfr(cond - unc)));
        } else {
            v = rd(b);
        }
        if (out_dtype == 0) ((float*)out)[i] = v;
        else ((u16*)out)[i] = f2bf(v);
    }
}

template <bool BF>
__global__ void ode_combine_kernel(int mode, const void* y0, const void* k1, const void* k2, const void* k3,
                                   const void* k4, void* out, float dt, long long n) {
#pragma clang fp contract(off)
    const long long i = (long long)blockIdx.x * blockDim.x + threadIdx.x;
    if (i >= n) return;
    auto ld = [&](const void* p) { return BF ? bf2f(((const u16*)p)[i]) : ((const float*)p)[i]; };
    auto R = [](float x) { return BF ? bfr(x) : x; };
    const float y = ld(y0);
    float r;
    if (mode == 0) r = y + R(dt * ld(k1));
    else if (mode == 1) r = y + R(R(dt * ld(k1)) * (1.0f / 3.0f));
    else if (mode == 2) r = y + R(dt * R(ld(k2) - R(ld(k1) * (1.0f / 3.0f))));
    else if (mode == 3) r = y + R(dt * R(R(ld(k1) - ld(k2)) + ld(k3)));
    else r = y + R(R(R(R(ld(k1) + R(3.0f * R(ld(k2) + ld(k3)))) + ld(k4)) * dt) * 0.125f);
// ... 44 lines not shown
__global__ void fill_rows_bf16_kernel(u16* dst, const u16* row, long long rows, int d) {
    const long long total = rows * d;
    for (long long i = (long long)blockIdx.x * blockDim.x + threadIdx.x; i < total; i += (long long)gridDim.x * blockDim.x)
        dst[i] = row[i % d];
}

__global__ void region_text_combine_kernel(u16* __restrict__ out, const u16* __restrict__ txt, const u16* __restrict__ gate,
                                           int Y, int N, int H, int hd, int Hp, int Wp, int h_split, int w_split) {
    const int d = H * hd, chunks = d >> 3;
    const long long total = (long long)2 * N * chunks;
    const int hps = Hp / h_split, wps = Wp / w_split;
    for (long long i = (long long)blockIdx.x * blockDim.x + threadIdx.x; i < total; i += (long long)gridDim.x * blockDim.x) {
        const int c = (int)(i % chunks);
        const long long rown = i / chunks;
        const int b = (int)(rown / N), n = (int)(rown % N);
        const int head = (c * 8) / hd;
        const float g = bfr(tanhf(bf2f(gate[head])));
        float acc[8];
#pragma unroll
        for (int k = 0; k < 8; ++k) acc[k] = 0.f;
        if (b == 0) {
            const int gr = n / Wp, gc = n - gr * Wp;
            const int ci = hps > 0 ? gr / hps : h_split, cj = wps > 0 ? gc / wps : w_split;
            const int region = (ci < h_split && cj < w_split) ? (ci + 1) * (cj + 1) - 1 : -1;
            if (region >= 0 && region < Y - 1) {
                const bf8_t t = *(const bf8_t*)(txt + ((size_t)region * N + n) * d + c * 8);
#pragma unroll
                for (int k = 0; k < 4; ++k) {
                    const f32x2 v = unpk_bf(t.w[k]);
                    acc[2 * k] = bfr(v[0] * g);
                    acc[2 * k + 1] = bfr(v[1] * g);
                }
            }
        } else {
            const bf8_t t = *(const bf8_t*)(txt + ((size_t)(Y - 1) * N + n) * d + c * 8);
#pragma unroll
            for (int k = 0; k < 4; ++k) {
                const f32x2 v = unpk_bf(t.w[k]);
                acc[2 * k] = bfr(v[0] * g);
                acc[2 * k + 1] = bfr(v[1] * g);
            }
        }
        u16* o = out + ((size_t)b * N + n) * d + c * 8;
        bf8_t cur = *(const bf8_t*)o, res;
#pragma unroll
        for (int k = 0; k < 4; ++k) {
            const f32x2 v = unpk_bf(cur.w[k]);
            res.w[k] = pk_bf(f32x2{v[0] + acc[2 * k], v[1] + acc[2 * k + 1]});
        }
        *(bf8_t*)o = res;
    }
}

inline int nblk(long long n, int bs) { return (int)((n + bs - 1) / bs); }

}

int launch_linear_small_m(const u16* a, const u16* w, const u16* b, u16* y, int M, int N, int K, int act_in,
                          hipStream_t stream) {
    LT_REQUIRE(M >= 1 && M <= SM_MAXM, "linear_small_m: M=%d out of range 1..%d", M, SM_MAXM);
    LT_REQUIRE(K % 8 == 0, "linear_small_m: K=%d must be a multiple of 8", K);
    const dim3 grid(((N + SM_NC - 1) / SM_NC + 3) / 4);
    if (M <= 2) hipLaunchKernelGGL((linear_small_m_kernel<2, false>), grid, dim3(256), 0, stream, a, w, b, y, M, N, K, act_in, LinearSmallMExtra());
    else if (M <= 4) hipLaunchKernelGGL((linear_small_m_kernel<4, false>), grid, dim3(256), 0, stream, a, w, b, y, M, N, K, act_in, LinearSmallMExtra());
    else hipLaunchKernelGGL((linear_small_m_kernel<8, false>), grid, dim3(256), 0, stream, a, w, b, y, M, N, K, act_in, LinearSmallMExtra());
    LT_CHECK_HIP(hipGetLastError());
    return 0;
}

int launch_linear_small_m_ext(const u16* a, const u16* w, const u16* b, u16* y, int M, int N, int K, int act_in, const LinearSmallMExtra& x,
                              hipStream_t stream) {
    LT_REQUIRE(M >= 1 && M <= SM_MAXM, "linear_small_m: M=%d out of range 1..%d", M, SM_MAXM);
    LT_REQUIRE(K % 8 == 0 && (!x.t || K % 16 == 0), "linear_small_m: K=%d must be a multiple of 8 (16 with timestep features)", K);
    LT_REQUIRE(a || x.t, "linear_small_m: no input");
    LT_REQUIRE(x.pm_d == 0 || (x.pm_L > 0 && x.pm_chunks > 0 && x.pm_chunks <= 32), "linear_small_m: bad prep_mod geometry");
    const dim3 grid(((N + SM_NC - 1) / SM_NC + 3) / 4);
    if (M <= 2) hipLaunchKernelGGL((linear_small_m_kernel<2, true>), grid, dim3(256), 0, stream, a, w, b, y, M, N, K, act_in, x);
    else if (M <= 4) hipLaunchKernelGGL((linear_small_m_kernel<4, true>), grid, dim3(256), 0, stream, a, w, b, y, M, N, K, act_in, x);
    else hipLaunchKernelGGL((linear_small_m_kernel<8, true>), grid, dim3(256), 0, stream, a, w, b, y, M, N, K, act_in, x);
    LT_CHECK_HIP(hipGetLastError());
    return 0;
}

int launch_cast_to_bf16(const void* src, int dtype, u16* dst, long long n, hipStream_t stream) {
    LT_REQUIRE(dtype >= 0 && dtype <= 2, "cast_to_bf16: bad dtype %d", dtype);
    if (n == 0) return 0;
    int g = nblk(n, 256);
    if (g > 8192) g = 8192;
    hipLaunchKernelGGL(cast_to_bf16_kernel, dim3(g), dim3(256), 0, stream, src, dtype, dst, n);
    LT_CHECK_HIP(hipGetLastError());
    return 0;
}

int launch_patchify(const void* x, int x_dtype, u16* out, int B, int C, int H, int W, int patch, int kpad,
                    int dup_first_half, int wp_stride, hipStream_t stream) {
    LT_REQUIRE(H % patch == 0 && W % patch == 0, "patchify: %dx%d not divisible by patch %d", H, W, patch);
    LT_REQUIRE(C * patch * patch <= kpad, "patchify: kpad too small");
    LT_REQUIRE(!dup_first_half || B % 2 == 0, "patchify: CFG needs an even batch");
    const long long total = (long long)B * (H / patch) * (W / patch) * kpad;
    int g = nblk(total, 256);
    if (g > 8192) g = 8192;
    hipLaunchKernelGGL(patchify_kernel, dim3(g), dim3(256), 0, stream, x, x_dtype, out, B, C, H, W, patch, kpad,
                       dup_first_half, wp_stride > 0 ? wp_stride : W / patch);
    LT_CHECK_HIP(hipGetLastError());
    return 0;
}

int launch_timestep_features(const float* t, int t_index, u16* out, int B, int dim, hipStream_t stream) {
    LT_REQUIRE(dim % 2 == 0, "timestep_features: odd dim unsupported");
    hipLaunchKernelGGL(timestep_features_kernel, dim3(nblk((long long)B * dim / 2, 128)), dim3(128), 0, stream,
                       t + (size_t)t_index * B, out, B, dim);
    LT_CHECK_HIP(hipGetLastError());
    return 0;
}

int launch_cap_pool_ln(const void* cap, int cap_dtype, const int32_t* mask, const u16* ln_w, const u16* ln_b, u16* out,
                       int B, int T, int C, hipStream_t stream) {
    hipLaunchKernelGGL(cap_pool_ln_kernel, dim3(B), dim3(256), (C + 8) * sizeof(float), stream, cap, cap_dtype, mask,
                       ln_w, ln_b, out, T, C);
    LT_CHECK_HIP(hipGetLastError());
    return 0;
}

int launch_prep_mod(u16* mod, int B, int ld_mod, int L, int chunks, int d, unsigned tanh_mask, unsigned scale_mask,
                    int final_scale_chunk, hipStream_t stream) {
    const long long total = (long long)B * ((long long)L * chunks * d + d);
    int g = nblk(total, 256);
    if (g > 4096) g = 4096;
    hipLaunchKernelGGL(prep_mod_kernel, dim3(g), dim3(256), 0, stream, mod, B, ld_mod, L, chunks, d, tanh_mask, scale_mask,
                       final_scale_chunk);
    LT_CHECK_HIP(hipGetLastError());
    return 0;
}

int launch_add_bf16(const u16* a, const u16* b, u16* c, long long n, hipStream_t stream) {
    hipLaunchKernelGGL(add_bf16_kernel, dim3(nblk(n, 256)), dim3(256), 0, stream, a, b, c, n);
    LT_CHECK_HIP(hipGetLastError());
    return 0;
}

int launch_mask_to_bias(const int32_t* mask, float* bias, int B, int T, int Tpad, hipStream_t stream) {
    hipLaunchKernelGGL(mask_to_bias_kernel, dim3(nblk((long long)B * Tpad, 256)), dim3(256), 0, stream, mask, bias, B,
                       T, Tpad);
    LT_CHECK_HIP(hipGetLastError());
    return 0;
}

int launch_unpatchify_cfg(const u16* rows, int ld, void* out, int out_dtype, int B, int C, int out_ch, int H, int W,
                          int patch, int use_cfg, float cfg_scale, int cfg_channels, int wp_stride, hipStream_t stream) {
    LT_REQUIRE(!use_cfg || B % 2 == 0, "unpatchify_cfg: CFG needs an even batch");
    const long long total = (long long)B * C * H * W;
    int g = nblk(total, 256);
    if (g > 8192) g = 8192;
    hipLaunchKernelGGL(unpatchify_cfg_kernel, dim3(g), dim3(256), 0, stream, rows, ld, out, out_dtype, B, C, out_ch, H,
                       W, patch, use_cfg, cfg_scale, cfg_channels, wp_stride > 0 ? wp_stride : W / patch);
    LT_CHECK_HIP(hipGetLastError());
    return 0;
}

int launch_unpatchify_cfg_dev(const u16* rows, int ld, void* out, int out_dtype, int B, int C, int out_ch, int H, int W, int patch, int use_cfg,
                              const float* cfg_scale_dev, int cfg_channels, int wp_stride, int dup, hipStream_t stream) {
    LT_REQUIRE(rows && out, "unpatchify_cfg_dev: null argument");
    LT_REQUIRE(B >= 1 && C >= 1 && out_ch >= C && patch >= 1 && H >= patch && W >= patch && H % patch == 0 && W % patch == 0 &&
               ld >= patch * patch * out_ch, "unpatchify_cfg_dev: bad shape");
    LT_REQUIRE(!(use_cfg || dup) || B % 2 == 0, "unpatchify_cfg_dev: guidance and dup need an even count of output rows");
    LT_REQUIRE(dup || !use_cfg || cfg_scale_dev, "unpatchify_cfg_dev: null scale");
// ... 153 lines not shown
```

### lumina-t2x_amd/csrc/ops_abi.hip

```cpp
#include <cstdio>
#include <cstring>

#include "../../include/lumina_dit.h"
#include "../../include/lumina_dit_debug.h"
#include "common.h"
#include "kernels.h"
#include "options.h"

extern "C" int lt_op_gemm_bf16(const void* A, const void* W, const void* bias, int32_t bias_dtype, void* C, int32_t M,
                               int32_t N, int32_t K, int32_t epilogue, int32_t variant, void* stream) {
    LT_REQUIRE(A && W && C, "lt_op_gemm_bf16: null pointer");
    GemmArgs g;
    g.A = (const u16*)A; g.W = (const u16*)W; g.C = (u16*)C; g.bias = bias; g.M = M; g.N = N; g.K = K;
    g.lda = K; g.ldw = K; g.ldc = epilogue == 1 ? N / 2 : N; g.bias_dtype = bias ? bias_dtype : -1;
    return launch_gemm_bf16(g, epilogue, variant, (hipStream_t)stream);
}

extern "C" int lt_op_pair_layout(void* m, int64_t rows, int32_t cols, int32_t to_pair, void* stream) {
    LT_REQUIRE(m, "lt_op_pair_layout: null pointer");
    return launch_pair_layout((u16*)m, rows, cols, to_pair, (hipStream_t)stream);
}
extern "C" int lt_op_gemm_bf16_pair(const void* A, const void* W, void* C, int32_t M, int32_t N, int32_t K, int32_t epilogue, int32_t pair_c,
                                    void* stream) {
    LT_REQUIRE(A && W && C, "lt_op_gemm_bf16_pair: null pointer");
// ... 438 lines not shown
    return launch_attention(a, (hipStream_t)stream);
}

extern "C" int lt_op_attention_qraw_ex(const void* qkv, int32_t ld, int32_t q_col0, const void* q_mean_rstd, const void* q_ln_w, const void* q_ln_b,
                                       const void* cs_table, const void* cs_table_t, int32_t table_len, int32_t grid_w, const void* t_dev,
                                       float watershed, const void* k, const void* vt, const void* tk, const void* tvt, const float* tbias,
                                       const void* tgate, int32_t Tk, int32_t Tkpad, void* out, int32_t B, int32_t H, int32_t Hkv, int32_t N,
                                       int32_t Nkpad, int32_t hd, void* stream) {
    return attention_qraw_ex("lt_op_attention_qraw_ex", qkv, ld, q_col0, q_mean_rstd, q_ln_w, q_ln_b, cs_table, cs_table_t, table_len, grid_w, t_dev, watershed, k, vt,
                             tk, tvt, tbias, tgate, Tk, Tkpad, out, B, H, Hkv, N, Nkpad, hd, nullptr, stream);
}

extern "C" int lt_op_attention_qraw_nk(const void* qkv, int32_t ld, int32_t q_col0, const void* q_mean_rstd, const void* q_ln_w, const void* q_ln_b,
                                       const void* cs_table, const void* cs_table_t, int32_t table_len, int32_t grid_w, const void* t_dev,
                                       float watershed, const void* k, const void* vt, const void* tk, const void* tvt, const float* tbias,
                                       const void* tgate, int32_t Tk, int32_t Tkpad, void* out, int32_t B, int32_t H, int32_t Hkv, int32_t N,
                                       int32_t Nkpad, int32_t hd, const int32_t* nk, void* stream) {
    return attention_qraw_ex("lt_op_attention_qraw_nk", qkv, ld, q_col0, q_mean_rstd, q_ln_w, q_ln_b, cs_table, cs_table_t, table_len, grid_w, t_dev, watershed, k, vt,
                             tk, tvt, tbias, tgate, Tk, Tkpad, out, B, H, Hkv, N, Nkpad, hd, nk, stream);
}

extern "C" int lt_op_attention_small(const void* qkv, int32_t ld, int32_t q_col0, int32_t k_col0, int32_t v_col0, const void* rowstat, int32_t slots,
                                     int32_t q_slot0, int32_t q_nslot, int32_t k_slot0, int32_t k_nslot, const void* q_ln_w, const void* q_ln_b,
                                     const void* k_ln_w, const void* k_ln_b, const void* cs_table, int32_t table_len, int32_t grid_w,
                                     const void* t_dev, float watershed, float k_scale, void* out, int32_t B, int32_t H, int32_t Hkv,
                                     int32_t tokens, int32_t hd, void* stream) {
    LT_REQUIRE(qkv && rowstat && q_ln_w && q_ln_b && k_ln_w && k_ln_b && cs_table && out, "lt_op_attention_small: null pointer");
    LT_REQUIRE(B > 0 && H > 0 && Hkv > 0 && hd > 0 && tokens > 0, "lt_op_attention_small: bad shape");
    AttnSmallArgs a;
    a.qkv = (const u16*)qkv; a.ld = ld; a.q_col0 = q_col0; a.k_col0 = k_col0; a.v_col0 = v_col0;
    a.rowstat = (const float*)rowstat; a.slots = slots; a.q_slot0 = q_slot0; a.q_nslot = q_nslot; a.k_slot0 = k_slot0; a.k_nslot = k_nslot;
    a.q_ln_w = (const u16*)q_ln_w; a.q_ln_b = (const u16*)q_ln_b; a.k_ln_w = (const u16*)k_ln_w; a.k_ln_b = (const u16*)k_ln_b; a.ln_eps = 1e-5f;
    a.cs = (const float*)cs_table; a.t = (const float*)t_dev; a.watershed = watershed; a.cs_len = table_len; a.grid_w = grid_w;
    a.k_scale = k_scale; a.out = (u16*)out; a.B = B; a.H = H; a.Hkv = Hkv; a.N = tokens; a.hd = hd;
    return launch_attention_small(a, (hipStream_t)stream);
}

extern "C" int lt_op_qkv_attention_small(const void* A, const void* W, void* qkv, int32_t M, int32_t K, int32_t H, int32_t Hkv, int32_t tokens,
                                         int32_t hd, const void* q_ln_w, const void* q_ln_b, const void* k_ln_w, const void* k_ln_b,
                                         const void* cs_table, int32_t table_len, int32_t grid_w, float k_scale, void* rowstat_ws,
                                         void* out, void* stream) {
    LT_REQUIRE(A && W && qkv && q_ln_w && q_ln_b && k_ln_w && k_ln_b && cs_table && rowstat_ws && out, "lt_op_qkv_attention_small: null pointer");
    LT_REQUIRE(H > 0 && Hkv > 0 && hd > 0 && tokens > 0 && M > 0 && M % tokens == 0, "lt_op_qkv_attention_small: bad shape");
    const int d = H * hd, dkv = Hkv * hd, N = d + 2 * dkv;
    LT_REQUIRE(attention_small_fusable(hd, tokens, H, Hkv, d, dkv), "lt_op_qkv_attention_small: head_dim 48, 64 <= tokens <= 512 in whole tiles, widths %% 128 == 0");
    GemmArgs g;
    g.A = (const u16*)A; g.W = (const u16*)W; g.C = (u16*)qkv; g.bias = nullptr; g.bias_dtype = -1; g.M = M; g.N = N; g.K = K;
    g.lda = K; g.ldw = K; g.ldc = N;
    LT_REQUIRE(gemm_is_small_m(g, 0), "lt_op_qkv_attention_small: %d x %d x %d does not run on the small-M tiles", M, N, K);
    g.rowstat = (float*)rowstat_ws; g.rowstat_slots = (N + 127) / 128;
    if (launch_gemm_bf16(g, 0, 0, (hipStream_t)stream)) return 1;
    AttnSmallArgs a;
    a.qkv = (const u16*)qkv; a.ld = N; a.q_col0 = 0; a.k_col0 = d; a.v_col0 = d + dkv;
    a.rowstat = (const float*)rowstat_ws; a.slots = g.rowstat_slots; a.q_slot0 = 0; a.q_nslot = d / 128; a.k_slot0 = d / 128; a.k_nslot = dkv / 128;
    a.q_ln_w = (const u16*)q_ln_w; a.q_ln_b = (const u16*)q_ln_b; a.k_ln_w = (const u16*)k_ln_w; a.k_ln_b = (const u16*)k_ln_b; a.ln_eps = 1e-5f;
    a.cs = (const float*)cs_table; a.t = nullptr; a.watershed = 0.f; a.cs_len = table_len; a.grid_w = grid_w;
    a.k_scale = k_scale; a.out = (u16*)out; a.B = M / tokens; a.H = H; a.Hkv = Hkv; a.N = tokens; a.hd = hd;
    return launch_attention_small(a, (hipStream_t)stream);
}

extern "C" int lt_op_attention_fused(const void* q, const void* k, const void* vt, const void* tk, const void* tvt,
                                     const float* tbias, const void* tgate, void* out, int32_t B, int32_t H, int32_t Hkv, int32_t N,
                                     int32_t Nk, int32_t Nkpad, int32_t Tk, int32_t Tkpad, int32_t hd, void* stream) {
    LT_REQUIRE(q && k && vt && tk && tvt && tbias && tgate && out, "lt_op_attention_fused: null pointer");
    LT_REQUIRE(attention_fuses_text(hd), "lt_op_attention_fused: needs head_dim 72 or 96 and attention_variant 3 or 4");
    AttnArgs a;
    a.q = (const u16*)q; a.k = (const u16*)k; a.vt = (const u16*)vt; a.bias = nullptr; a.out = (u16*)out; a.gate = nullptr;
    a.accumulate = 0; a.B = B; a.H = H; a.Hkv = Hkv; a.N = N; a.Nk = Nk; a.Nkpad = Nkpad; a.hd = hd; a.scale = 1.f; a.k_prescaled = 1;
    a.tk = (const u16*)tk; a.tvt = (const u16*)tvt; a.tbias = tbias; a.tgate = (const u16*)tgate; a.Tk = Tk; a.Tkpad = Tkpad;
    return launch_attention(a, (hipStream_t)stream);
}

extern "C" int lt_op_attention_trace(const void* q, const void* k, const void* vt, void* out, int32_t B, int32_t H, int32_t Hkv,
                                     int32_t N, int32_t Nk, int32_t Nkpad, int32_t hd, float scale, void* trace_dev,
                                     void* stream) {
    LT_REQUIRE(q && k && vt && out && trace_dev, "lt_op_attention_trace: null pointer");
    AttnArgs a;
    a.q = (const u16*)q; a.k = (const u16*)k; a.vt = (const u16*)vt; a.bias = nullptr; a.out = (u16*)out;
    a.gate = nullptr; a.accumulate = 0; a.B = B; a.H = H; a.Hkv = Hkv; a.N = N; a.Nk = Nk;
    a.Nkpad = Nkpad; a.hd = hd; a.scale = scale; a.trace = (unsigned long long*)trace_dev;
    return launch_attention(a, (hipStream_t)stream);
}

extern "C" int lt_op_linear_small_m(const void* a, const void* w, const void* b, void* y, int32_t M, int32_t N, int32_t K,
                                    int32_t act_in, void* stream) {
    LT_REQUIRE(a && w && y, "lt_op_linear_small_m: null pointer");
    return launch_linear_small_m((const u16*)a, (const u16*)w, (const u16*)b, (u16*)y, M, N, K, act_in, (hipStream_t)stream);
}

extern "C" int lt_op_rope_table_2d_pair(void* out, void* out_t, int32_t len, int32_t hd, float theta, float scale_factor, void* stream) {
    LT_REQUIRE(out && out_t, "lt_op_rope_table_2d_pair: null pointer");
    return launch_rope_table_2d((float*)out, len, hd, theta, scale_factor, (hipStream_t)stream, (float*)out_t);
}

extern "C" int lt_op_rope_table_2d(void* out, int32_t len, int32_t hd, float theta, float scale_factor, void* stream) {
    LT_REQUIRE(out, "lt_op_rope_table_2d: null pointer");
    return launch_rope_table_2d((float*)out, len, hd, theta, scale_factor, (hipStream_t)stream);
}

extern "C" int lt_op_views_invert(const int32_t* perm_dev, int32_t* iperm_dev, int32_t* hits_dev, int32_t V, int32_t HW, void* stream) {
    return launch_views_invert(perm_dev, iperm_dev, hits_dev, V, HW, (hipStream_t)stream);
}
extern "C" int lt_op_views_gather(const void* y_dev, const int32_t* perm_dev, const float* vsign_dev, const void* f0_dev, void* out_dev, float half_dt,
                                  int32_t V, int32_t C, int32_t HW, int32_t dtype, void* stream) {
    return launch_views_gather(y_dev, perm_dev, vsign_dev, f0_dev, out_dev, half_dt, V, C, HW, dtype, (hipStream_t)stream);
}
extern "C" int lt_op_views_reduce(const void* y_dev, const void* f_dev, const int32_t* iperm_dev, const float* isign_dev, void* out_dev, float dt,
                                  int32_t V, int32_t C, int32_t HW, int32_t dtype, void* stream) {
    return launch_views_reduce(y_dev, f_dev, iperm_dev, isign_dev, out_dev, dt, V, C, HW, dtype, (hipStream_t)stream);
}
extern "C" int lt_op_windows_gather(const void* y_dev, const int32_t* offsets_host, int32_t n, int32_t win_h, int32_t win_w, int32_t canvas_h,
                                    int32_t canvas_w, void* out_dev, int32_t C, int32_t dtype, void* stream) {
    WindowTable t;
    if (window_table_build("lt_op_windows_gather", offsets_host, n, win_h, win_w, canvas_h, canvas_w, &t)) return 2;
    return launch_windows_gather(y_dev, t, out_dev, C, dtype, (hipStream_t)stream);
}
extern "C" int lt_op_windows_reduce(const void* f_dev, const int32_t* offsets_host, int32_t n, int32_t win_h, int32_t win_w, int32_t canvas_h,
                                    int32_t canvas_w, const float* weight_dev, const float* wsum_dev, void* out_dev, int32_t C, int32_t dtype,
                                    void* stream) {
    WindowTable t;
    if (window_table_build("lt_op_windows_reduce", offsets_host, n, win_h, win_w, canvas_h, canvas_w, &t)) return 2;
    return launch_windows_reduce(f_dev, t, weight_dev, wsum_dev, out_dev, C, dtype, (hipStream_t)stream);
}
extern "C" int lt_op_windows_cover(const int32_t* offsets_host, int32_t n, int32_t win_h, int32_t win_w, int32_t canvas_h, int32_t canvas_w,
                                   const float* weight_dev, float* wsum_dev, int32_t* bad_dev, void* stream) {
    WindowTable t;
    if (window_table_build("lt_op_windows_cover", offsets_host, n, win_h, win_w, canvas_h, canvas_w, &t)) return 2;
    return launch_windows_cover(t, weight_dev, wsum_dev, bad_dev, (hipStream_t)stream);
}
extern "C" int lt_op_views_guided_gather(const void* y_dev, const void* guidance_dev, const void* noise_dev, const int32_t* perm_dev,
                                         const float* vsign_dev, const float* isign_dev, const void* f0_dev, void* out_dev, float half_dt,
                                         const float* coef_host, int32_t V, int32_t C, int32_t HW, int32_t dtype, void* stream) {
    return launch_views_guided_gather(y_dev, guidance_dev, noise_dev, perm_dev, vsign_dev, isign_dev, f0_dev, out_dev, half_dt, coef_host, V, C, HW, dtype,
                                      (hipStream_t)stream);
}

extern "C" int lt_op_sde_step(int32_t op, const void* x_dev, const void* v_dev, const void* w_dev, const void* k1_dev, const void* xp_dev,
                              void* out_dev, void* out2_dev, const float* rec_host, int64_t n, int32_t dtype, void* stream) {
    return launch_sde_step(op, x_dev, v_dev, w_dev, k1_dev, xp_dev, out_dev, out2_dev, rec_host, (long long)n, dtype, (hipStream_t)stream);
}

extern "C" int lt_op_flowedit_mix(const void* x_src_dev, const void* z_dev, const void* noise_dev, void* out4_dev, float t, float one_minus_t,
                                  int64_t n_half, int32_t dtype, void* stream) {
    return launch_flowedit_mix(x_src_dev, z_dev, noise_dev, out4_dev, t, one_minus_t, (long long)n_half, dtype, (hipStream_t)stream);
}
extern "C" int lt_op_flowedit_combine(const void* z_dev, const void* out4_dev, void* z_next_dev, float w_s, float w_t, float dt, int32_t Bp, int32_t C,
                                      int32_t HW, int32_t ch, int32_t dtype, void* stream) {
    return launch_flowedit_combine(z_dev, out4_dev, z_next_dev, w_s, w_t, dt, Bp, C, HW, ch, dtype, (hipStream_t)stream);
}

extern "C" int lt_op_rk_stage(const void* y_dev, const void* const* k_ptrs_host, const float* coef_host, int32_t nk, float dt, void* out_dev,
                              int64_t n, int32_t dtype, void* stream) {
    return launch_rk_stage(y_dev, k_ptrs_host, coef_host, nk, dt, out_dev, (long long)n, dtype, (hipStream_t)stream);
}
extern "C" int lt_op_rk_error_norm(const void* y_dev, const void* y1_dev, const void* const* k_ptrs_host, const float* coef_host, int32_t nk,
                                   float dt, float rtol, float atol, void* q_dev, void* ws_dev, float* norm_dev, int64_t n, int32_t dtype,
                                   void* stream) {
    return launch_rk_error_norm(y_dev, y1_dev, k_ptrs_host, coef_host, nk, dt, rtol, atol, q_dev, ws_dev, norm_dev, (long long)n, dtype,
                                (hipStream_t)stream);
}
extern "C" int lt_op_rk_dense(const void* y_dev, const void* y1_dev, const void* ymid_dev, const void* fy_dev, const void* f1_dev, float dt,
                              void* c1_dev, void* c_dev, void* b_dev, void* a_dev, int64_t n, int32_t dtype, void* stream) {
    return launch_rk_dense(y_dev, y1_dev, ymid_dev, fy_dev, f1_dev, dt, c1_dev, c_dev, b_dev, a_dev, (long long)n, dtype, (hipStream_t)stream);
}
extern "C" int lt_op_rk_interp(const void* const* coef_ptrs_host, float x, void* out_dev, int64_t n, int32_t dtype, void* stream) {
    return launch_rk_interp(coef_ptrs_host, x, out_dev, (long long)n, dtype, (hipStream_t)stream);
// ... 186 lines not shown
```

### lumina-t2x_amd/csrc/options.h

```cpp
#pragma once
#include <atomic>
#include <climits>

enum LtOpt {
    OPT_GRAPH = 0, OPT_ATTENTION_VARIANT, OPT_QKV_POST_FUSED, OPT_QKV_VT_EPILOGUE, OPT_QKV_FUSED_GEMM, OPT_QK_POST_PAIR, OPT_ATTN_Q_FUSED,
    OPT_NORM_SPECIALIZE, OPT_GEMM_W4Q, OPT_GEMM_PREFETCH, OPT_GEMM_SPLITK, OPT_GEMM_W4Q_GROUPED, OPT_GEMM_GROUP, OPT_GEMM_STAGGER,
    OPT_GEMM_VARIANT, OPT_RMSNORM_APEX, OPT_ATTN_SMALL_FUSED, OPT_MOE_ROUTE_FUSED, OPT_GEMM_SPLITK4, OPT_MOE_TIME_PLAN_HOIST,
    OPT_GRN_YSTAT, OPT_QK_WG_PER_CU, OPT_PROLOGUE_FUSED, OPT_GEMM_TAIL_SPLIT, OPT_ATTN_TEXT_SKIP, OPT_ATTN_TAIL_SPLIT, OPT_PAIR_LAYOUT,
    LT_OPT_COUNT
};
constexpr int LT_OPT_INHERIT = INT_MIN;

struct LtOptDesc {
    const char* name;
    int lo, hi, def;
    bool boolean;
};
extern const LtOptDesc kLtOptDesc[LT_OPT_COUNT];

int lt_opt_find(const char* name);
int lt_opt(int id);
int lt_opt_generation();
int lt_opt_engine_generation();
int lt_opt_validate(int id, int* value);
void lt_opt_set_process(int id, int value);
void lt_opt_reset_process();

struct LtEngineOptions {
    std::atomic<int> v[LT_OPT_COUNT];
    std::atomic<int> gen{0};
    LtEngineOptions() { for (int i = 0; i < LT_OPT_COUNT; ++i) v[i].store(LT_OPT_INHERIT, std::memory_order_relaxed); }
};
struct LtOptScope {
    int v[LT_OPT_COUNT];
    int process_gen, engine_gen;
    const LtOptScope* prev;
    explicit LtOptScope(const LtEngineOptions* o);
    ~LtOptScope();
    LtOptScope(const LtOptScope&) = delete;
    LtOptScope& operator=(const LtOptScope&) = delete;
};
```

### lumina-t2x_amd/csrc/options.hip

```cpp
#include <atomic>
#include <cstring>

#include "common.h"
#include "kernels.h"
#include "options.h"

const LtOptDesc kLtOptDesc[LT_OPT_COUNT] = {
    {"graph", 0, 2, 2, false},
    {"attention_variant", 1, 6, 4, false},
    {"qkv_post_fused", 0, 2, 2, false},
    {"qkv_vt_epilogue", 0, 1, 1, true},
    {"qkv_fused_gemm", 0, 1, 1, true},
    {"qk_post_pair", 0, 1, 1, true},
    {"attn_q_fused", 0, 1, 1, true},
    {"norm_specialize", 0, 1, 1, true},
    {"gemm_w4q", 0, 1, 1, true},
    {"gemm_prefetch", 0, 3, 3, false},
    {"gemm_splitk", 0, 2, 1, false},
    {"gemm_w4q_grouped", 0, 2, 1, false},
    {"gemm_group", 0, 64, 0, false},
    {"gemm_stagger", 0, 256, 0, false},
    {"gemm_variant", 0, 2, 0, false},
    {"rmsnorm_apex", 0, 1, 0, true},
    {"attn_small_fused", 0, 1, 1, true},
    {"moe_route_fused", 0, 1, 1, true},
    {"gemm_splitk4", 0, 1, 1, true},
    {"moe_time_plan_hoist", 0, 1, 1, true},
    {"grn_ystat", 0, 2, 1, false},
    {"qk_wg_per_cu", 1, 8, 3, false},
    {"prologue_fused", 0, 7, 0, false},
    {"gemm_tail_split", 0, 2, 0, false},
    {"attn_text_skip", 0, 1, 1, true},
    {"attn_tail_split", 0, 4, 4, false},
    {"pair_layout", 0, 1, 1, true},
};

namespace {
struct ProcessOptions {
    std::atomic<int> v[LT_OPT_COUNT];
    std::atomic<int> gen{0};
    ProcessOptions() { for (int i = 0; i < LT_OPT_COUNT; ++i) v[i].store(kLtOptDesc[i].def, std::memory_order_relaxed); }
};
ProcessOptions& process() {
    static ProcessOptions p;
    return p;
}
thread_local const LtOptScope* tl_scope = nullptr;
}

int lt_opt_find(const char* name) {
    if (!name) return -1;
    for (int i = 0; i < LT_OPT_COUNT; ++i)
        if (strcmp(name, kLtOptDesc[i].name) == 0) return i;
    return -1;
}

int lt_opt(int id) {
    if (tl_scope) return tl_scope->v[id];
    return process().v[id].load(std::memory_order_relaxed);
}

int lt_opt_generation() { return tl_scope ? tl_scope->process_gen : process().gen.load(std::memory_order_relaxed); }
int lt_opt_engine_generation() { return tl_scope ? tl_scope->engine_gen : 0; }

int lt_opt_validate(int id, int* value) {
    const LtOptDesc& d = kLtOptDesc[id];
    if (d.boolean) { *value = *value != 0; return 0; }
    if (id == OPT_ATTENTION_VARIANT && *value == 5) {
        lt_set_error("attention_variant 5 (PV on 16x16x32 MFMAs) was a study kernel of csrc/experimental/, removed in round 5 (it lost on issue slots, NOTEBOOK.md 5.8)");
        return 2;
    }
    if (id == OPT_GEMM_PREFETCH && *value == 2) {
        lt_set_error("gemm_prefetch 2 (weight-panel reads on a side stream) lost 33 %% in its A/B and was removed in round 5; use 0, 1 or 3");
        return 2;
    }
    if (*value < d.lo || *value > d.hi) {
        lt_set_error("option %s must be %d .. %d (got %d)", d.name, d.lo, d.hi, *value);
        return 2;
    }
    return 0;
}

void lt_opt_set_process(int id, int value) {
    process().v[id].store(value, std::memory_order_relaxed);
    process().gen.fetch_add(1, std::memory_order_release);
}

void lt_opt_reset_process() {
    for (int i = 0; i < LT_OPT_COUNT; ++i) process().v[i].store(kLtOptDesc[i].def, std::memory_order_relaxed);
    process().gen.fetch_add(1, std::memory_order_release);
}

LtOptScope::LtOptScope(const LtEngineOptions* o) : prev(tl_scope) {
    process_gen = process().gen.load(std::memory_order_acquire);
    engine_gen = o ? o->gen.load(std::memory_order_acquire) : 0;
    for (int i = 0; i < LT_OPT_COUNT; ++i) {
        const int ov = o ? o->v[i].load(std::memory_order_relaxed) : LT_OPT_INHERIT;
        v[i] = ov != LT_OPT_INHERIT ? ov : process().v[i].load(std::memory_order_relaxed);
    }
    tl_scope = this;
}
LtOptScope::~LtOptScope() { tl_scope = prev; }
```

### lumina-t2x_amd/csrc/samplers.hip

```cpp
#include <algorithm>
#include <cmath>
#include <cstring>
#include <vector>

#include "engine.h"
#include "guidance_plan.h"
#include "kernels.h"

namespace {

int check_latent(const lt_engine* e, const char* who, int h, int w) {
    const int p = e->cfg.patch_size;
    LT_REQUIRE(h > 0 && w > 0 && h % p == 0 && w % p == 0 && (long long)(h / p) * (w / p) <= e->cfg.max_tokens,
               "%s: latent %dx%d is not a positive multiple of the patch size or exceeds max_tokens %d", who, h, w, e->cfg.max_tokens);
    return 0;
}

int check_step_shape(const lt_engine* e, const char* who, const lt_step_args* a) {
    LT_REQUIRE(a->batch >= 1 && a->batch <= e->cfg.max_batch, "%s: batch %d outside 1..max_batch %d", who, a->batch, e->cfg.max_batch);
    if (check_latent(e, who, a->latent_h, a->latent_w)) return 2;
    LT_REQUIRE(a->io_dtype == LT_BF16 || a->io_dtype == LT_F32, "io_dtype must be bf16 or f32");
    return 0;
}

// ... 88 lines not shown
        for (int k = 0; k < st.n_kinds; ++k) rows += lt_eval_traits(st.kinds[k]).half ? a->batch / 2 : a->batch;
        if (st.n_kinds == 2) {
            ++nfe;
            return forward_slg_pair(e, "skip-layer guidance", plan, y, t, out, a, s, st.kinds[1], scale,
                                    e->times.dev + GuidancePlan::second_offset(ncalls, a->batch) + call);
        }
        return forward_rewriting(e, st.rewrites, y, t, out, a, lt_eval_traits(st.kinds[0]).dev_scale ? 1 : use_cfg, s, {st.kinds[0], pc, scale});
    }
    int eval_cached(const void* y, const float* t, int call, void* out) {
        CacheControl* cache = plan.cache;
        bool run = true;
        double rel = 0.0;
        if (call > 0 && call < ncalls - 1) {
            if (int rc = cache_probe(e, y, t, a, use_cfg, s)) return rc;
            run = cache->step(e->c_sums_host[0], e->c_sums_host[1], &rel);
        } else if (int rc = forward_graphed(e, y, t, nullptr, a, use_cfg, s, {LT_KIND_CACHE_HEAD})) {
            return rc;
        }
        if (cache->stats) { cache->stats[3 * call] = rel; cache->stats[3 * call + 1] = cache->acc; cache->stats[3 * call + 2] = run ? 1.0 : 0.0; }
        if (!run) {
            ++hits;
            return forward_graphed(e, y, t, out, a, use_cfg, s, {LT_KIND_CACHE_APPLY});
        }
        cache->acc = 0.0;
        rows += a->batch;
        return forward_rewriting(e, LT_STORED_RESIDUAL, y, t, out, a, use_cfg, s, {LT_KIND_CACHE_BLOCKS});
    }
    int advance(int traj_slot) {
        if (traj) LT_CHECK_HIP(hipMemcpyAsync((char*)traj + (size_t)traj_slot * sbytes, y1(), sbytes, hipMemcpyDeviceToDevice, s));
        cur ^= 1;
        return 0;
    }
    int finish(void* final_dev) {
        if (final_dev) LT_CHECK_HIP(hipMemcpyAsync(final_dev, y0(), sbytes, hipMemcpyDeviceToDevice, s));
        e->last_nfe = nfe;
        e->last_eval_rows = rows;
        if (plan.form == LT_PLAN_CACHED) e->last_cache_hits = hits;
        e->layout_flips = e->layout_flips_total - flips0;
        return 0;
    }
};

float bf16_round_host(float f) {
    uint32_t u;
    memcpy(&u, &f, 4);
    u += 0x7fffu + ((u >> 16) & 1u);
    u &= 0xffff0000u;
    memcpy(&f, &u, 4);
    return f;
}

struct GridCall {
    const void* z; void *traj, *final;
    const float* tgrid; int n_grid, use_cfg, t_round;
    const lt_step_args* a; hipStream_t s; long long n; const PackedCall* pc;
    int method = 0; const float* coef = nullptr; int corrector = 0;
    bool tiled = false;
};
struct MaskedBlend { const void *mask, *x1, *noise; };

long long dense_elems(const lt_engine* e, const lt_step_args* a) { return (long long)a->batch * e->cfg.in_channels * a->latent_h * a->latent_w; }

int apply_plan(lt_engine* e, const GuidancePlan& plan, const lt_step_args* a, int ncalls, hipStream_t s) {
    const float* second = e->times.dev + GuidancePlan::second_offset(ncalls, a->batch);
    if (plan.projected()) LT_CHECK_HIP(hipMemcpyAsync(e->p_par + 1, second, 3 * sizeof(float), hipMemcpyDeviceToDevice, s));
    if (plan.form == LT_PLAN_PROJECT_APG && zero_momentum(e, a, s)) return 1;
    if (plan.form == LT_PLAN_RULE) LT_CHECK_HIP(hipMemcpyAsync(e->g_cfg + 1, second, 2 * sizeof(float), hipMemcpyDeviceToDevice, s));
    return 0;
}

int ode_fixed_grid(lt_engine* e, const GridCall& c, const GuidancePlan& plan, const MaskedBlend* mb) {
    const lt_step_args* a = c.a;
    hipStream_t s = c.s;
    const float* tgrid_host = c.tgrid;
    const int B = a->batch, n_grid = c.n_grid, method = c.method;
    const long long n = c.n;
    const int stages = method == LT_ODE_EULER ? 1 : (method == LT_ODE_MIDPOINT ? 2 : 4);
    const int ncalls = (n_grid - 1) * stages;
    const bool bf = a->io_dtype == LT_BF16;
    const int nsent = ncalls * B + plan.tail_floats(ncalls);
    float* tp = e->times.begin(nsent, s);
    if (!tp) return 1;
    std::vector<float> dts(n_grid - 1);
    for (int i = 0; i + 1 < n_grid; ++i) {
        const float t0 = tgrid_host[i], t1 = tgrid_host[i + 1];
        const float dt = t1 - t0;
        dts[i] = dt;
        float ts[4];
        if (method == LT_ODE_EULER) ts[0] = t0;
        else if (method == LT_ODE_MIDPOINT) { ts[0] = t0; ts[1] = t0 + 0.5f * dt; }
        else { ts[0] = t0; ts[1] = t0 + dt * (float)(1.0 / 3.0); ts[2] = t0 + dt * (float)(2.0 / 3.0); ts[3] = t1; }
        for (int k = 0; k < stages; ++k) {
            const float tv = (c.t_round && bf) ? bf16_round_host(ts[k]) : ts[k];
            for (int b = 0; b < B; ++b) tp[((size_t)i * stages + k) * B + b] = tv;
        }
    }
    plan.fill_tail(tp + GuidancePlan::table_offset(ncalls, B), ncalls);
    if (e->times.commit(nsent, s) || apply_plan(e, plan, a, ncalls, s)) return 1;
    Trajectory tr{e, a, c.use_cfg, s, (size_t)n * (bf ? 2 : 4), c.pc, plan, ncalls};
    if (tr.start(c.z, c.traj, true)) return 1;
    const int dt_code = bf ? 1 : 0;
    auto eval = [&](const void* y, int call, void* out) -> int {
        if (!c.tiled) return tr.eval(y, call, out);
        if (launch_windows_gather(y, e->tw, e->tw_in, e->cfg.in_channels, dt_code, s)) return 1;
        if (tr.eval(e->tw_in, call, e->tw_out)) return 1;
        return launch_windows_reduce(e->tw_out, e->tw, e->tw_has_weight ? e->tw_weight : nullptr, e->tw_wsum, out, e->cfg.in_channels, dt_code, s);
    };
    for (int i = 0; i + 1 < n_grid; ++i) {
        void *y0 = tr.y0(), *y1 = tr.y1();
        if (i < plan.zero_init) {
            if (tr.traj) LT_CHECK_HIP(hipMemcpyAsync((char*)tr.traj + (size_t)(i + 1) * tr.sbytes, y0, tr.sbytes, hipMemcpyDeviceToDevice, s));
            continue;
        }
        const float dt = bf ? bf16_round_host(dts[i]) : dts[i];
        const int c0 = i * stages;
        auto close = [&](int mode, const void* k1, const void* k2, const void* k3, const void* k4) -> int {
            if (!mb) return launch_ode_combine(mode, y0, k1, k2, k3, k4, y1, dt_code, dt, n, s);
            const float t1 = tgrid_host[i + 1];
            return launch_ode_combine_masked(mode, y0, k1, k2, k3, k4, mb->mask, mb->x1, mb->noise, y1, dt_code, dt, t1, (float)(1.0 - (double)t1), n, s);
        };
        if (method == LT_ODE_EULER) {
            if (eval(y0, c0, e->kbuf[0])) return 1;
            if (close(0, e->kbuf[0], nullptr, nullptr, nullptr)) return 1;
        } else if (method == LT_ODE_MIDPOINT) {
            if (eval(y0, c0, e->kbuf[0])) return 1;
            if (launch_ode_combine(0, y0, e->kbuf[0], nullptr, nullptr, nullptr, e->ymid, dt_code, 0.5f * dt, n, s)) return 1;
            if (eval(e->ymid, c0 + 1, e->kbuf[1])) return 1;
            if (close(0, e->kbuf[1], nullptr, nullptr, nullptr)) return 1;
        } else {
            if (eval(y0, c0, e->kbuf[0])) return 1;
            if (launch_ode_combine(1, y0, e->kbuf[0], nullptr, nullptr, nullptr, e->ymid, dt_code, dt, n, s)) return 1;
            if (eval(e->ymid, c0 + 1, e->kbuf[1])) return 1;
            if (launch_ode_combine(2, y0, e->kbuf[0], e->kbuf[1], nullptr, nullptr, e->ymid, dt_code, dt, n, s)) return 1;
            if (eval(e->ymid, c0 + 2, e->kbuf[2])) return 1;
            if (launch_ode_combine(3, y0, e->kbuf[0], e->kbuf[1], e->kbuf[2], nullptr, e->ymid, dt_code, dt, n, s)) return 1;
            if (eval(e->ymid, c0 + 3, e->kbuf[3])) return 1;
            if (close(4, e->kbuf[0], e->kbuf[1], e->kbuf[2], e->kbuf[3])) return 1;
        }
        if (tr.advance(i + 1)) return 1;
    }
    return tr.finish(c.final);
}

}

static int sample_plain(lt_engine* e, const char* who, GridCall c, const int32_t* hw_host, bool packed, const MaskedBlend* mb) {
    LT_REQUIRE(!mb || (mb->mask && mb->x1 && mb->noise), "%s: null mask, source or noise", who);
    LT_REQUIRE(e && c.z && c.tgrid && c.a && (hw_host || !packed), "%s: null argument", who);
    if (refuse_if_capturing(c.s, who)) return 2;
    LtOptScope opt_scope(&e->opts);
    if (check_grid_method(who, c.n_grid, c.method, mb != nullptr, "")) return 2;
    PackedCall pc{};
    if (packed) {
        if (int rc = packed_call_begin(e, who, hw_host, c.a, c.use_cfg, &pc, c.s)) return rc;
        c.n = pc.elems; c.pc = &pc;
    } else {
        if (check_step_shape(e, who, c.a)) return 2;
        LT_REQUIRE(!mb || !c.use_cfg || c.a->batch % 2 == 0, "%s: guidance needs an even batch (cond + uncond rows), got %d", who, c.a->batch);
        c.n = dense_elems(e, c.a);
    }
    return ode_fixed_grid(e, c, {}, mb);
}

extern "C" int lt_sample_ode(lt_engine* e, const void* z_dev, void* traj_dev, void* final_dev, const float* tgrid_host,
                             int32_t n_grid, int32_t method, int32_t use_cfg, int32_t t_round, const lt_step_args* a,
                             void* stream) {
    return sample_plain(e, "lt_sample_ode", {z_dev, traj_dev, final_dev, tgrid_host, n_grid, use_cfg, t_round, a, (hipStream_t)stream, 0, nullptr, method}, nullptr,
                        false, nullptr);
}

static int check_cached_call(lt_engine* e, const char* who, const lt_step_args* a, int use_cfg) {
    if (check_step_shape(e, who, a)) return 2;
    LT_REQUIRE(!use_cfg || a->batch % 2 == 0, "%s: guidance needs an even batch (cond + uncond rows), got %d", who, a->batch);
    LT_REQUIRE(e->reg_Y == 0, "%s: a regional prompt is prepared (lt_prepare_prompt_regional): step caching does not serve it", who);
    LT_REQUIRE(!e->moe_rec_on && !e->moe_force_rows, "%s: MoE routing record / force is on: step caching does not serve it", who);
    LT_REQUIRE(e->skip.empty(), "%s: a layer-skip set is not served", who);
    LT_REQUIRE(e->prompt_B == a->batch, "%s: %s was called for batch %d, step has batch %d", who, e->v.labels ? "lt_prepare_labels" : "lt_prepare_prompt",
               e->prompt_B, a->batch);
    return 0;
}

extern "C" int lt_sample_ode_cached(lt_engine* e, const void* z_dev, void* traj_dev, void* final_dev, const float* tgrid_host, int32_t n_grid,
                                    int32_t method, int32_t use_cfg, int32_t t_round, const lt_step_args* a, float threshold,
                                    const double* coef_host, double* stats_host, void* stream) {
    LT_REQUIRE(e && z_dev && tgrid_host && a && coef_host, "lt_sample_ode_cached: null argument");
// ... 1006 lines not shown
```

Measured before the change: 147,900.

## Hoist timestep conditioning across ODE evaluations into batched row GEMVs

Before the fixed-grid ODE loop, the timestep-embedding and adaLN modulation chain is precomputed for a window of upcoming evaluations in one batched pass (up to 64 rows), using a new weight-stationary linear_rows kernel. Each evaluation then copies its slice into the live conditioning buffers instead of running several small-M GEMV launches over the full adaLN weight matrix. This removes repeated weight reads and kernel launches per step. In exchange it adds extra buffers, a copy kernel per evaluation, and a new graph-cache key dimension, and it applies only to whole evaluations with no guidance plan.

```diff
diff --git a/include/lumina_dit_debug.h b/include/lumina_dit_debug.h
--- a/include/lumina_dit_debug.h
+++ b/include/lumina_dit_debug.h
@@ -115,6 +115,8 @@
 int lt_op_linear_small_m_ext(const void* a, const void* w, const void* b, void* y, int32_t M, int32_t N, int32_t K, int32_t act_in, const void* t,
                              const void* a2, int32_t pm_L, int32_t pm_chunks, int32_t pm_d, int32_t pm_final, uint32_t pm_tanh, uint32_t pm_scale,
                              void* stream);
+int lt_op_linear_rows(const void* a, const void* a2, int32_t a2_rows, const void* w, const void* b, void* y, void* act, int32_t R, int32_t N,
+                      int32_t K, int32_t act_in, void* stream);
 int lt_op_moe_route(const void* x, const void* gate_w, const void* forced, int32_t rows, int32_t rows_per_sample, int32_t d, int32_t E, void* sel,
                     void* wts, int32_t max_tiles, void* stream);
 int lt_op_moe_plan_ex(void* sel, const void* sample_logits, int32_t sample_ld, const void* forced, void* wts, int32_t rows,
diff --git a/lumina-t2x_amd/_lib.py b/lumina-t2x_amd/_lib.py
--- a/lumina-t2x_amd/_lib.py
+++ b/lumina-t2x_amd/_lib.py
@@ -231,6 +231,7 @@
     "lt_op_ode_multistep": (_i32, [_vp, C.POINTER(_vp), _i32, C.POINTER(_f32), C.POINTER(_f32), _i32, _vp, _vp, _i64, _i32, _vp]),
     "lt_op_rope_table": (_i32, [_vp, _i32, _i32, _i32, _f32, _f32, _f32, _f32, _i32, _vp, _vp]),
     "lt_op_linear_small_m_ext": (_i32, [_vp, _vp, _vp, _vp, _i32, _i32, _i32, _i32, _vp, _vp, _i32, _i32, _i32, _i32, C.c_uint32, C.c_uint32, _vp]),
+    "lt_op_linear_rows": (_i32, [_vp, _vp, _i32, _vp, _vp, _vp, _vp, _i32, _i32, _i32, _i32, _vp]),
     "lt_op_moe_route": (_i32, [_vp, _vp, _vp, _i32, _i32, _i32, _i32, _vp, _vp, _i32, _vp]),
     "lt_op_moe_plan_ex": (_i32, [_vp, _vp, _i32, _vp, _vp, _i32, _i32, _i32, _vp, _vp, _vp, _i32, _i32, _i64, _i64, _i64, _vp]),
     "lt_op_rope_table_2d": (_i32, [_vp, _i32, _i32, _f32, _f32, _vp]),
diff --git a/lumina-t2x_amd/csrc/engine.h b/lumina-t2x_amd/csrc/engine.h
--- a/lumina-t2x_amd/csrc/engine.h
+++ b/lumina-t2x_amd/csrc/engine.h
@@ -8,6 +8,7 @@
 #include "eval_kind.h"
 #include "kernels.h"
 #include "options.h"
+#include "stage_times.h"
 
 struct DevBuf {
     void* p = nullptr;
@@ -100,6 +101,13 @@
         if (norm_host) (void)hipHostFree(norm_host);
         ws = nullptr; norm_dev = nullptr; norm_host = nullptr;
     }
+};
+
+constexpr int LT_COND_HOIST_MAX_ROWS = 64;
+struct CondHoist {
+    u16 *tfeat = nullptr, *t1 = nullptr, *temb = nullptr, *act = nullptr, *logits = nullptr, *mod = nullptr;
+    CondHoistWindow win;
+    int row = -1, B = 0;
 };
 
 struct lt_engine {
@@ -158,6 +166,7 @@
     int softmax_rule = LT_SOFTMAX_T2I;
     void *ys[2] = {nullptr, nullptr}, *ymid = nullptr, *kbuf[4] = {nullptr, nullptr, nullptr, nullptr};
     StageTimes times;
+    CondHoist hoist;
     RkWork rk;
     int reg_Y = 0, reg_h = 1, reg_w = 1;
     u16* reg_txt = nullptr;
@@ -236,6 +245,19 @@
     ~SkipScope() { e->skip.clear(); e->perturb.clear(); }
     int set(const char* who, const int32_t* skip_host, int n_skip, const int32_t* perturb_host = nullptr, int n_perturb = 0);
 };
+struct CondHoistScope {
+    lt_engine* e;
+    const lt_step_args* a = nullptr;
+    hipStream_t s = nullptr;
+    int ncalls = 0, cap_rows = 0;
+    bool on = false;
+    explicit CondHoistScope(lt_engine* eng) : e(eng) {}
+    CondHoistScope(const CondHoistScope&) = delete;
+    CondHoistScope& operator=(const CondHoistScope&) = delete;
+    ~CondHoistScope() { e->hoist.row = -1; }
+    int begin(const lt_step_args* a, int ncalls, hipStream_t s);
+    int before(int call);
+};
 int check_layer_sets(const lt_engine* e, const char* who, const int32_t* skip_host, int n_skip, const int32_t* perturb_host, int n_perturb);
 int check_skip_set(const lt_engine* e, const char* who, const int32_t* skip_host, int n_skip);
 bool stream_capturing(hipStream_t s);
diff --git a/lumina-t2x_amd/csrc/engine.hip b/lumina-t2x_amd/csrc/engine.hip
--- a/lumina-t2x_amd/csrc/engine.hip
+++ b/lumina-t2x_amd/csrc/engine.hip
@@ -479,31 +479,45 @@
     return 0;
 }
 
+void prep_mod_masks(const lt_engine* e, unsigned* tanh_mask, unsigned* scale_mask, int* fin2) {
+    const VariantDesc& v = e->v;
+    *tanh_mask = 0; *scale_mask = 0;
+    for (int i = 0; i < 2; ++i) {
+        if (v.gate_tanh && v.i_gate[i] >= 0) *tanh_mask |= 1u << v.i_gate[i];
+        if (v.i_scale[i] >= 0) *scale_mask |= 1u << v.i_scale[i];
+    }
+    if (e->cfg.variant == LT_VARIANT_NEXT_MOE) { *tanh_mask |= 1u << 5; *scale_mask |= 1u << 4; }
+    *fin2 = v.final_chunks == 2 ? 1 : 0;
+}
+
+int moe_time_plans(lt_engine* e, const Dims& dm, hipStream_t s) {
+    MoeArgs m;
+    m.x = nullptr; m.gate_w = nullptr; m.forced = nullptr; m.sample_logits = e->moe_logits; m.sample_ld = e->L * e->E;
+    m.rows = dm.M; m.rows_per_sample = dm.N; m.d = e->d; m.E = e->E;
+    m.sel = e->moe_tp_sel; m.pos = e->moe_tp_pos; m.wts = e->moe_tp_wts; m.src = e->moe_tp_src; m.tile_expert = e->moe_tp_tile_expert;
+    m.max_tiles = moe_tiles_for(e, dm.M);
+    m.layers = e->L; m.layer_stride_rows = (long long)e->moe_tp_stride_rows; m.layer_stride_src = (long long)e->moe_tp_stride_src; m.layer_stride_tiles = e->moe_tiles;
+    return launch_moe_plan(m, s);
+}
+
 int condition(lt_engine* e, const Dims& dm, const float* t_dev, hipStream_t s) {
-    const VariantDesc& v = e->v;
     const int B = dm.B, L = e->L, A = e->A;
+    if (e->hoist.row >= 0) {
+        LT_REQUIRE(B == e->hoist.B, "hoisted conditioning: prepared for %d rows, the evaluation has %d", e->hoist.B, B);
+        if (!e->moe_tp_live) return 0;
+        ProfScope ps(e, 2, 0, s);
+        return moe_time_plans(e, dm, s) ? 1 : 0;
+    }
     ProfScope ps(e, 2, 0, s);
     const int fused_pro = lt_opt(OPT_PROLOGUE_FUSED);
     if (fused_pro & 1) { LinearSmallMExtra x; x.t = t_dev; if (launch_linear_small_m_ext(nullptr, e->t0_w, e->t0_b, e->t1, B, A, 256, 0, x, s)) return 1; }
     else if (launch_timestep_features(t_dev, 0, e->tfeat, B, 256, s) || launch_linear_small_m(e->tfeat, e->t0_w, e->t0_b, e->t1, B, A, 256, 0, s)) return 1;
     if (launch_linear_small_m(e->t1, e->t2_w, e->t2_b, e->temb, B, A, A, 1, s)) return 1;
     if (e->gate_t_all && launch_linear_small_m(e->temb, e->gate_t_all, nullptr, e->moe_logits, B, L * e->E, A, 0, s)) return 1;
-    if (e->moe_tp_live) {
-        MoeArgs m;
-        m.x = nullptr; m.gate_w = nullptr; m.forced = nullptr; m.sample_logits = e->moe_logits; m.sample_ld = L * e->E;
-        m.rows = dm.M; m.rows_per_sample = dm.N; m.d = e->d; m.E = e->E;
-        m.sel = e->moe_tp_sel; m.pos = e->moe_tp_pos; m.wts = e->moe_tp_wts; m.src = e->moe_tp_src; m.tile_expert = e->moe_tp_tile_expert;
-        m.max_tiles = moe_tiles_for(e, dm.M);
-        m.layers = L; m.layer_stride_rows = (long long)e->moe_tp_stride_rows; m.layer_stride_src = (long long)e->moe_tp_stride_src; m.layer_stride_tiles = e->moe_tiles;
-        if (launch_moe_plan(m, s)) return 1;
-    }
-    unsigned tanh_mask = 0, scale_mask = 0;
-    for (int i = 0; i < 2; ++i) {
-        if (v.gate_tanh && v.i_gate[i] >= 0) tanh_mask |= 1u << v.i_gate[i];
-        if (v.i_scale[i] >= 0) scale_mask |= 1u << v.i_scale[i];
-    }
-    if (e->cfg.variant == LT_VARIANT_NEXT_MOE) { tanh_mask |= 1u << 5; scale_mask |= 1u << 4; }
-    const int fin2 = v.final_chunks == 2 ? 1 : 0;
+    if (e->moe_tp_live && moe_time_plans(e, dm, s)) return 1;
+    unsigned tanh_mask, scale_mask;
+    int fin2;
+    prep_mod_masks(e, &tanh_mask, &scale_mask, &fin2);
     LinearSmallMExtra x;
     const u16* in = e->temb;
     if (fused_pro & 2) x.a2 = e->cap_emb;
@@ -513,6 +527,30 @@
                       : launch_linear_small_m(in, e->adaln_w, e->adaln_b, e->mod, B, e->ld_mod, A, 1, s)) return 1;
     if (!(fused_pro & 4) && launch_prep_mod(e->mod, B, e->ld_mod, L, e->chunks, e->d, tanh_mask, scale_mask, fin2, s)) return 1;
     return 0;
+}
+
+int condition_rows(lt_engine* e, const float* t_dev, int R, int B, hipStream_t s) {
+    const int L = e->L, A = e->A;
+    CondHoist& h = e->hoist;
+    ProfScope ps(e, 2, 0, s);
+    if (launch_timestep_features(t_dev, 0, h.tfeat, R, 256, s)) return 1;
+    if (launch_linear_rows(h.tfeat, nullptr, 0, e->t0_w, e->t0_b, h.t1, h.act, R, A, 256, 0, s)) return 1;
+    if (launch_linear_rows(h.t1, nullptr, 0, e->t2_w, e->t2_b, h.temb, h.act, R, A, A, 1, s)) return 1;
+    if (e->gate_t_all && launch_linear_rows(h.temb, nullptr, 0, e->gate_t_all, nullptr, h.logits, h.act, R, L * e->E, A, 0, s)) return 1;
+    if (launch_linear_rows(h.temb, e->cap_emb, B, e->adaln_w, e->adaln_b, h.mod, h.act, R, e->ld_mod, A, 1, s)) return 1;
+    unsigned tanh_mask, scale_mask;
+    int fin2;
+    prep_mod_masks(e, &tanh_mask, &scale_mask, &fin2);
+    return launch_prep_mod(h.mod, R, e->ld_mod, L, e->chunks, e->d, tanh_mask, scale_mask, fin2, s) ? 1 : 0;
+}
+
+int condition_place(lt_engine* e, hipStream_t s) {
+    const CondHoist& h = e->hoist;
+    const size_t r = (size_t)h.row;
+    const u16* src[3] = {h.mod + r * e->ld_mod, h.temb + r * e->A, e->gate_t_all ? h.logits + r * e->L * e->E : nullptr};
+    u16* dst[3] = {e->mod, e->temb, e->gate_t_all ? e->moe_logits : nullptr};
+    const long long words[3] = {(long long)h.B * e->ld_mod, (long long)h.B * e->A, (long long)h.B * e->L * e->E};
+    return launch_cond_copy(src, dst, words, s);
 }
 
 bool fuses_text(const lt_engine* e) { return e->v.text && !(e->reg_Y > 0) && attention_fuses_text(e->hd); }
@@ -947,6 +985,12 @@
         a = &own;
         use_cfg = kt.half ? 0 : 1;
     }
+    const bool hoisted = e->hoist.row >= 0;
+    if (hoisted) {
+        LT_REQUIRE(kind == LT_KIND_WHOLE && a->batch == e->hoist.B, "hoisted conditioning: an evaluation of kind %d on %d rows inside a trajectory "
+                   "prepared for whole evaluations on %d rows", (int)kind, a->batch, e->hoist.B);
+        if (condition_place(e, s)) return 1;
+    }
     auto run = [&](const void* x, const float* t, void* o, hipStream_t st) {
         if (!pc) return run_forward(e, x, t, o, a, use_cfg, st, nullptr, kind);
         PackedDesc pk{nullptr, nullptr, pc->hw};
@@ -965,8 +1009,8 @@
     const size_t cap_bytes = (size_t)e->cfg.max_batch * e->cfg.in_channels * e->cfg.max_tokens * e->cfg.patch_size * e->cfg.patch_size * 4;
     if ((kt.half ? 2 * sbytes : sbytes) > cap_bytes) return run(x_in, t_dev, out, s);
     if (stream_capturing(s)) return run(x_in, t_dev, out, s);
-    const int extra[11] = {use_cfg, e->prompt_B, e->prompt_T, e->prompt_Tpad, e->reg_Y, e->reg_h, e->reg_w, lt_opt_generation(), lt_opt_engine_generation(),
-                           e->softmax_rule, (int)kind};
+    const int extra[12] = {use_cfg, e->prompt_B, e->prompt_T, e->prompt_Tpad, e->reg_Y, e->reg_h, e->reg_w, lt_opt_generation(), lt_opt_engine_generation(),
+                           e->softmax_rule, (int)kind, hoisted ? 1 : 0};
     std::vector<char> key(sizeof(lt_step_args) + sizeof(extra));
     memcpy(key.data(), a, sizeof(lt_step_args));
     memcpy(key.data() + sizeof(lt_step_args), extra, sizeof(extra));
@@ -1055,6 +1099,48 @@
     const int rc = forward_graphed_body(e, x_in, t_dev, out, a, use_cfg, s, spec);
     if (rc == 0 && spec.kind == LT_KIND_CACHE_HEAD) memcpy(e->cache_head, sig, sizeof sig);
     return rc;
+}
+
+static int cond_hoist_reserve(lt_engine* e) {
+    CondHoist& h = e->hoist;
+    if (h.mod) return 0;
+    const size_t R = LT_COND_HOIST_MAX_ROWS, A = e->A;
+    void* q = nullptr;
+    if (dev_alloc(e, &q, R * 256 * sizeof(u16), false)) return 1;
+    h.tfeat = (u16*)q;
+    if (dev_alloc(e, &q, R * A * sizeof(u16), false)) return 1;
+    h.t1 = (u16*)q;
+    if (dev_alloc(e, &q, R * A * sizeof(u16), false)) return 1;
+    h.temb = (u16*)q;
+    if (dev_alloc(e, &q, R * std::max<size_t>(A, 256) * sizeof(u16), false)) return 1;
+    h.act = (u16*)q;
+    if (e->gate_t_all) { if (dev_alloc(e, &q, R * e->L * e->E * sizeof(u16), false)) return 1; h.logits = (u16*)q; }
+    if (dev_alloc(e, &q, R * e->ld_mod * sizeof(u16), false)) return 1;
+    h.mod = (u16*)q;
+    return 0;
+}
+
+int CondHoistScope::begin(const lt_step_args* a_, int ncalls_, hipStream_t s_) {
+    a = a_; s = s_; ncalls = ncalls_;
+    cap_rows = std::min(lt_opt(OPT_COND_HOIST), LT_COND_HOIST_MAX_ROWS);
+    e->hoist.row = -1;
+    on = cap_rows > 0 && ncalls > 0 && e->weights_ok && a->batch >= 1 && a->batch <= cap_rows && a->batch <= e->cfg.max_batch && e->prompt_B == a->batch;
+    if (!on) return 0;
+    if (cond_hoist_reserve(e)) return 1;
+    e->hoist.B = a->batch;
+    e->hoist.win = CondHoistWindow{};
+    return 0;
+}
+
+int CondHoistScope::before(int call) {
+    if (!on) return 0;
+    CondHoist& h = e->hoist;
+    if (!h.win.holds(call)) {
+        h.win = CondHoistWindow::at(call, ncalls, h.B, cap_rows);
+        if (condition_rows(e, e->times.dev + h.win.time_index(0, h.B), h.win.count * h.B, h.B, s)) return 1;
+    }
+    h.row = h.win.row_of(call, h.B);
+    return 0;
 }
 
 int ensure_step_cache(lt_engine* e) {
diff --git a/lumina-t2x_amd/csrc/kernels.h b/lumina-t2x_amd/csrc/kernels.h
--- a/lumina-t2x_amd/csrc/kernels.h
+++ b/lumina-t2x_amd/csrc/kernels.h
@@ -230,6 +230,9 @@
 };
 int launch_linear_small_m_ext(const u16* a, const u16* w, const u16* b, u16* y, int M, int N, int K, int act_in,
                               const LinearSmallMExtra& x, hipStream_t stream);
+int launch_linear_rows(const u16* a, const u16* a2, int a2_rows, const u16* w, const u16* b, u16* y, u16* act, int R, int N, int K, int act_in,
+                       hipStream_t stream);
+int launch_cond_copy(const u16* const src[3], u16* const dst[3], const long long words[3], hipStream_t stream);
 int launch_cast_to_bf16(const void* src, int dtype, u16* dst, long long n, hipStream_t stream);
 int launch_patchify(const void* x, int x_dtype, u16* out, int B, int C, int H, int W, int patch, int kpad,
                     int dup_first_half, int wp_stride, hipStream_t stream);
diff --git a/lumina-t2x_amd/csrc/misc.hip b/lumina-t2x_amd/csrc/misc.hip
--- a/lumina-t2x_amd/csrc/misc.hip
+++ b/lumina-t2x_amd/csrc/misc.hip
@@ -1,3 +1,5 @@
+#include <algorithm>
+
 #include "common.h"
 #include "kernels.h"
 
@@ -223,6 +225,85 @@
 __global__ void add_bf16_kernel(const u16* a, const u16* b, u16* c, long long n) {
     const long long i = (long long)blockIdx.x * blockDim.x + threadIdx.x;
     if (i < n) c[i] = f2bf(bf2f(a[i]) + bf2f(b[i]));
+}
+
+__global__ void cond_rows_act_kernel(const u16* __restrict__ a, const u16* __restrict__ a2, int a2_rows, u16* __restrict__ out, int R, int K,
+                                     int act_in) {
+    const int r = blockIdx.y, k = blockIdx.x * blockDim.x + threadIdx.x;
+    if (r >= R || k >= K) return;
+    const size_t i = (size_t)r * K + k;
+    float v = bf2f(a[i]);
+    if (a2) v = bfr(v + bf2f(a2[(size_t)(r % a2_rows) * K + k]));
+    if (act_in == 1) v = bfr(silu_f(v));
+    out[i] = f2bf(v);
+}
+
+template <int KC>
+__global__ __launch_bounds__(256) void linear_rows_kernel(const u16* __restrict__ a, const u16* __restrict__ w, const u16* __restrict__ bias,
+                                                          u16* __restrict__ y, int R, int N, int K) {
+    const int lane = threadIdx.x & 63;
+    const int n0 = (blockIdx.x * 4 + (threadIdx.x >> 6)) * SM_NC;
+    if (n0 >= N) return;
+    const int nch = K >> 3;
+    float wf[KC][SM_NC][8];
+#pragma unroll
+    for (int q = 0; q < KC; ++q) {
+        const int c = lane + 64 * q;
+#pragma unroll
+        for (int j = 0; j < SM_NC; ++j) {
+            const int n = n0 + j < N ? n0 + j : N - 1;
+            if (c < nch) {
+                unpack8(*(const bf8_t*)(w + (size_t)n * K + c * 8), wf[q][j]);
+            } else {
+#pragma unroll
+                for (int e = 0; e < 8; ++e) wf[q][j][e] = 0.f;
+            }
+        }
+    }
+    const bool vec = n0 + SM_NC <= N && N % SM_NC == 0;
+    for (int r = 0; r < R; ++r) {
+        float acc[SM_NC];
+#pragma unroll
+        for (int j = 0; j < SM_NC; ++j) acc[j] = 0.f;
+#pragma unroll
+        for (int q = 0; q < KC; ++q) {
+            const int c = lane + 64 * q;
+            if (c < nch) {
+                float af[8];
+                unpack8(*(const bf8_t*)(a + (size_t)r * K + c * 8), af);
+#pragma unroll
+                for (int j = 0; j < SM_NC; ++j)
+#pragma unroll
+                    for (int e = 0; e < 8; ++e) acc[j] = __builtin_fmaf(af[e], wf[q][j][e], acc[j]);
+            }
+        }
+        float o[SM_NC];
+#pragma unroll
+        for (int j = 0; j < SM_NC; ++j) {
+            float s = wave_sum(acc[j]);
+            if (bias && n0 + j < N) s += bf2f(bias[n0 + j]);
+            o[j] = s;
+        }
+        if (lane == 0) {
+            if (vec) {
+                *(bf8_t*)(y + (size_t)r * N + n0) = pack8(o);
+            } else {
+#pragma unroll
+                for (int j = 0; j < SM_NC; ++j)
+                    if (n0 + j < N) y[(size_t)r * N + n0 + j] = f2bf(o[j]);
+            }
+        }
+    }
+}
+
+struct CondCopy { const u16* src[3]; u16* dst[3]; long long n16[3], words[3]; };
+__global__ void cond_copy_kernel(CondCopy c) {
+    const long long stride = (long long)gridDim.x * blockDim.x, i0 = (long long)blockIdx.x * blockDim.x + threadIdx.x;
+#pragma unroll
+    for (int k = 0; k < 3; ++k) {
+        for (long long i = i0; i < c.n16[k]; i += stride) ((bf8_t*)c.dst[k])[i] = ((const bf8_t*)c.src[k])[i];
+        for (long long i = c.n16[k] * 8 + i0; i < c.words[k]; i += stride) c.dst[k][i] = c.src[k][i];
+    }
 }
 
 __global__ void mask_to_bias_kernel(const int32_t* mask, float* bias, int B, int T, int Tpad) {
@@ -433,6 +514,45 @@
     return 0;
 }
 
+int launch_linear_rows(const u16* a, const u16* a2, int a2_rows, const u16* w, const u16* b, u16* y, u16* act, int R, int N, int K, int act_in,
+                       hipStream_t stream) {
+    LT_REQUIRE(R >= 1 && N >= 1 && K >= 8 && K % 8 == 0, "linear_rows: R=%d N=%d K=%d (K a positive multiple of 8)", R, N, K);
+    LT_REQUIRE(!a2 || a2_rows >= 1, "linear_rows: a2 without rows");
+    const u16* in = a;
+    if (a2 || act_in == 1) {
+        LT_REQUIRE(act, "linear_rows: no buffer for the prepared inputs");
+        hipLaunchKernelGGL(cond_rows_act_kernel, dim3(nblk(K, 256), R), dim3(256), 0, stream, a, a2, a2_rows, act, R, K, act_in);
+        LT_CHECK_HIP(hipGetLastError());
+        in = act;
+    }
+    if (K > 1024) {
+        for (int r = 0; r < R; r += SM_MAXM)
+            if (launch_linear_small_m(in + (size_t)r * K, w, b, y + (size_t)r * N, std::min(SM_MAXM, R - r), N, K, 0, stream)) return 1;
+        return 0;
+    }
+    const dim3 grid(((N + SM_NC - 1) / SM_NC + 3) / 4);
+    if (K <= 512) hipLaunchKernelGGL((linear_rows_kernel<1>), grid, dim3(256), 0, stream, in, w, b, y, R, N, K);
+    else hipLaunchKernelGGL((linear_rows_kernel<2>), grid, dim3(256), 0, stream, in, w, b, y, R, N, K);
+    LT_CHECK_HIP(hipGetLastError());
+    return 0;
+}
+
+int launch_cond_copy(const u16* const src[3], u16* const dst[3], const long long words[3], hipStream_t stream) {
+    CondCopy c;
+    long long most = 0;
+    for (int k = 0; k < 3; ++k) {
+        c.src[k] = src[k]; c.dst[k] = dst[k]; c.words[k] = src[k] && dst[k] ? words[k] : 0;
+        c.n16[k] = (((uintptr_t)src[k] | (uintptr_t)dst[k]) & 15) == 0 ? c.words[k] / 8 : 0;
+        most = std::max(most, c.n16[k] > 0 ? c.n16[k] : c.words[k]);
+    }
+    if (most == 0) return 0;
+    int g = nblk(most, 256);
+    if (g > 1024) g = 1024;
+    hipLaunchKernelGGL(cond_copy_kernel, dim3(g), dim3(256), 0, stream, c);
+    LT_CHECK_HIP(hipGetLastError());
+    return 0;
+}
+
 int launch_cast_to_bf16(const void* src, int dtype, u16* dst, long long n, hipStream_t stream) {
     LT_REQUIRE(dtype >= 0 && dtype <= 2, "cast_to_bf16: bad dtype %d", dtype);
     if (n == 0) return 0;
diff --git a/lumina-t2x_amd/csrc/ops_abi.hip b/lumina-t2x_amd/csrc/ops_abi.hip
--- a/lumina-t2x_amd/csrc/ops_abi.hip
+++ b/lumina-t2x_amd/csrc/ops_abi.hip
@@ -544,6 +544,13 @@
     return launch_attention(a, (hipStream_t)stream);
 }
 
+extern "C" int lt_op_linear_rows(const void* a, const void* a2, int32_t a2_rows, const void* w, const void* b, void* y, void* act, int32_t R, int32_t N,
+                                 int32_t K, int32_t act_in, void* stream) {
+    LT_REQUIRE(a && w && y, "lt_op_linear_rows: null pointer");
+    return launch_linear_rows((const u16*)a, (const u16*)a2, a2_rows, (const u16*)w, (const u16*)b, (u16*)y, (u16*)act, R, N, K, act_in,
+                              (hipStream_t)stream);
+}
+
 extern "C" int lt_op_linear_small_m(const void* a, const void* w, const void* b, void* y, int32_t M, int32_t N, int32_t K,
                                     int32_t act_in, void* stream) {
     LT_REQUIRE(a && w && y, "lt_op_linear_small_m: null pointer");
diff --git a/lumina-t2x_amd/csrc/options.h b/lumina-t2x_amd/csrc/options.h
--- a/lumina-t2x_amd/csrc/options.h
+++ b/lumina-t2x_amd/csrc/options.h
@@ -7,6 +7,7 @@
     OPT_NORM_SPECIALIZE, OPT_GEMM_W4Q, OPT_GEMM_PREFETCH, OPT_GEMM_SPLITK, OPT_GEMM_W4Q_GROUPED, OPT_GEMM_GROUP, OPT_GEMM_STAGGER,
     OPT_GEMM_VARIANT, OPT_RMSNORM_APEX, OPT_ATTN_SMALL_FUSED, OPT_MOE_ROUTE_FUSED, OPT_GEMM_SPLITK4, OPT_MOE_TIME_PLAN_HOIST,
     OPT_GRN_YSTAT, OPT_QK_WG_PER_CU, OPT_PROLOGUE_FUSED, OPT_GEMM_TAIL_SPLIT, OPT_ATTN_TEXT_SKIP, OPT_ATTN_TAIL_SPLIT, OPT_PAIR_LAYOUT,
+    OPT_COND_HOIST,
     LT_OPT_COUNT
 };
 constexpr int LT_OPT_INHERIT = INT_MIN;
diff --git a/lumina-t2x_amd/csrc/options.hip b/lumina-t2x_amd/csrc/options.hip
--- a/lumina-t2x_amd/csrc/options.hip
+++ b/lumina-t2x_amd/csrc/options.hip
@@ -33,6 +33,7 @@
     {"attn_text_skip", 0, 1, 1, true},
     {"attn_tail_split", 0, 4, 4, false},
     {"pair_layout", 0, 1, 1, true},
+    {"cond_hoist", 0, 64, 64, false},
 };
 
 namespace {
diff --git a/lumina-t2x_amd/csrc/samplers.hip b/lumina-t2x_amd/csrc/samplers.hip
--- a/lumina-t2x_amd/csrc/samplers.hip
+++ b/lumina-t2x_amd/csrc/samplers.hip
@@ -194,25 +194,16 @@
     float* tp = e->times.begin(nsent, s);
     if (!tp) return 1;
     std::vector<float> dts(n_grid - 1);
-    for (int i = 0; i + 1 < n_grid; ++i) {
-        const float t0 = tgrid_host[i], t1 = tgrid_host[i + 1];
-        const float dt = t1 - t0;
-        dts[i] = dt;
-        float ts[4];
-        if (method == LT_ODE_EULER) ts[0] = t0;
-        else if (method == LT_ODE_MIDPOINT) { ts[0] = t0; ts[1] = t0 + 0.5f * dt; }
-        else { ts[0] = t0; ts[1] = t0 + dt * (float)(1.0 / 3.0); ts[2] = t0 + dt * (float)(2.0 / 3.0); ts[3] = t1; }
-        for (int k = 0; k < stages; ++k) {
-            const float tv = (c.t_round && bf) ? bf16_round_host(ts[k]) : ts[k];
-            for (int b = 0; b < B; ++b) tp[((size_t)i * stages + k) * B + b] = tv;
-        }
-    }
+    lt_fixed_grid_times(tgrid_host, n_grid, method, c.t_round && bf, B, tp, dts.data());
     plan.fill_tail(tp + GuidancePlan::table_offset(ncalls, B), ncalls);
     if (e->times.commit(nsent, s) || apply_plan(e, plan, a, ncalls, s)) return 1;
+    CondHoistScope hoist(e);
+    if (plan.form == LT_PLAN_NONE && hoist.begin(a, ncalls, s)) return 1;
     Trajectory tr{e, a, c.use_cfg, s, (size_t)n * (bf ? 2 : 4), c.pc, plan, ncalls};
     if (tr.start(c.z, c.traj, true)) return 1;
     const int dt_code = bf ? 1 : 0;
     auto eval = [&](const void* y, int call, void* out) -> int {
+        if (hoist.before(call)) return 1;
         if (!c.tiled) return tr.eval(y, call, out);
         if (launch_windows_gather(y, e->tw, e->tw_in, e->cfg.in_channels, dt_code, s)) return 1;
         if (tr.eval(e->tw_in, call, e->tw_out)) return 1;
diff --git a/lumina-t2x_amd/csrc/stage_times.h b/lumina-t2x_amd/csrc/stage_times.h
--- /dev/null
+++ b/lumina-t2x_amd/csrc/stage_times.h
@@ -0,0 +1,45 @@
+#pragma once
+#include <cstdint>
+#include <cstring>
+
+constexpr int LT_STAGES_EULER = 1, LT_STAGES_MIDPOINT = 2, LT_STAGES_RK4 = 4;
+inline int lt_fixed_grid_stages(int method) { return method == 0 ? LT_STAGES_EULER : method == 1 ? LT_STAGES_MIDPOINT : LT_STAGES_RK4; }
+
+inline float lt_bf16_round_host(float f) {
+    uint32_t u;
+    memcpy(&u, &f, 4);
+    u += 0x7fffu + ((u >> 16) & 1u);
+    u &= 0xffff0000u;
+    memcpy(&f, &u, 4);
+    return f;
+}
+
+inline void lt_fixed_grid_times(const float* tgrid, int n_grid, int method, bool round_bf16, int B, float* times, float* dts) {
+    const int stages = lt_fixed_grid_stages(method);
+    for (int i = 0; i + 1 < n_grid; ++i) {
+        const float t0 = tgrid[i], t1 = tgrid[i + 1];
+        const float dt = t1 - t0;
+        dts[i] = dt;
+        float ts[4];
+        if (method == 0) ts[0] = t0;
+        else if (method == 1) { ts[0] = t0; ts[1] = t0 + 0.5f * dt; }
+        else { ts[0] = t0; ts[1] = t0 + dt * (float)(1.0 / 3.0); ts[2] = t0 + dt * (float)(2.0 / 3.0); ts[3] = t1; }
+        for (int k = 0; k < stages; ++k) {
+            const float tv = round_bf16 ? lt_bf16_round_host(ts[k]) : ts[k];
+            for (int b = 0; b < B; ++b) times[((size_t)i * stages + k) * B + b] = tv;
+        }
+    }
+}
+
+struct CondHoistWindow {
+    int first = 0, count = 0;
+    bool holds(int call) const { return call >= first && call < first + count; }
+    static CondHoistWindow at(int call, int ncalls, int B, int cap_rows) {
+        int n = B > 0 ? cap_rows / B : 0;
+        if (n < 1) n = 1;
+        if (n > ncalls - call) n = ncalls - call;
+        return {call, n};
+    }
+    int row_of(int call, int B) const { return (call - first) * B; }
+    size_t time_index(int row, int B) const { return (size_t)first * B + row; }
+};
```

Measured after the change: 148,300, median of 6. About the same (+0.3%).
